# Tezahc/image_processor_pipeline

Measured on AMD Instinct MI355X. Metric: Mpixels/sec through 5-stage pipe, 1024×1024 uint8; achieved HBM GB/s, higher is better.
Workload: dtype u8

## Files before the change

### image_processor_pipeline_amd/_native.py

```python
from __future__ import annotations

import ctypes
import os
from pathlib import Path

import numpy as np

LIB_PATH = Path(os.environ.get("IPP_LIB_PATH", str(Path(__file__).resolve().parent / "libipp.so")))
_EXPERIMENT = os.environ.get("IPP_AB_EXPERIMENT") == "1"

IPP_OK = 0
IPP_E_ARG = -1
IPP_E_LAUNCH = -2
IPP_E_RANGE = -3
IPP_MAX_HSV_RANGES = 16
IPP_TAPS_MFMA = 1
IPP_RS_PREMULTIPLY = 1
IPP_RS_UNPREMULTIPLY = 2


class NativeUnavailable(RuntimeError):
    """The HIP C-ABI library could not be loaded (never silently bypassed)."""


class NativeError(RuntimeError):
    pass


_I4 = np.int32
_I8 = np.int64

GATHER_DESC = np.dtype([
    ("src_off", _I8), ("dst_off", _I8), ("src_pitch", _I4), ("src_cn", _I4),
    ("src_w", _I4), ("src_h", _I4), ("in_x0", _I4), ("in_y0", _I4), ("in_w", _I4), ("in_h", _I4),
    ("a0", _I4), ("a1", _I4), ("a2", _I4), ("a3", _I4), ("a4", _I4), ("a5", _I4),
    ("out_w", _I4), ("out_h", _I4), ("off_x", _I4), ("off_y", _I4), ("flip", _I4), ("dst_pitch", _I4),
    ("base_off", _I8), ("lim", np.uint32), ("b", _I4, (6,)), ("prepared", _I4),
], align=True)

AFFINE_DESC = np.dtype([
    ("src_off", _I8), ("dst_off", _I8), ("src_pitch", _I4), ("src_cn", _I4),
    ("in_x0", _I4), ("in_y0", _I4), ("in_w", _I4), ("in_h", _I4),
    ("out_w", _I4), ("out_h", _I4), ("dst_pitch", _I4), ("flip", _I4), ("m", np.float64, (6,)),
], align=True)

IPP_ENH_BLUR = 1
IPP_ENH_LUT = 2
ENHANCE_DESC = np.dtype([
    ("src_off", _I8), ("dst_off", _I8), ("w", _I4), ("h", _I4), ("src_pitch", _I4), ("dst_pitch", _I4),
    ("f_brightness", np.float32), ("f_contrast", np.float32), ("f_color", np.float32), ("flags", _I4),
    ("box_r", _I4), ("box_ww", np.uint32), ("box_fw", np.uint32), ("pad_", _I4), ("lut_off", _I8),
], align=True)

COPY_DESC = np.dtype([
    ("src_off", _I8), ("dst_off", _I8), ("src_pitch", _I4), ("dst_pitch", _I4),
    ("x0", _I4), ("y0", _I4), ("w", _I4), ("h", _I4), ("cn", _I4), ("flip", _I4),
], align=True)

HSV_RANGE = np.dtype([("lo", _I4, (3,)), ("hi", _I4, (3,)), ("zone", _I4, (4,))], align=True)
HSV_PARAMS = np.dtype([("n_ranges", _I4), ("bgr", _I4), ("r", HSV_RANGE, (IPP_MAX_HSV_RANGES,))], align=True)

IMAGE_DESC = np.dtype([("off", _I8), ("w", _I4), ("h", _I4), ("pitch", _I4), ("cn", _I4)], align=True)

CCL_WORK = np.dtype([("mask_off", _I8), ("edge_off", _I8), ("p_off", _I8), ("a_off", _I8), ("ent_off", _I8), ("ent_cap", _I8),
                     ("tile_off", _I8), ("img_off", _I8)], align=True)

RESAMPLE_DESC = np.dtype([
    ("src_off", _I8), ("dst_off", _I8), ("src_pitch", _I4), ("dst_pitch", _I4),
    ("in_len", _I4), ("out_len", _I4), ("lines", _I4), ("line0", _I4), ("ksize", _I4), ("pad_", _I4),
    ("coef_off", _I8),
], align=True)

PASTE_DESC = np.dtype([
    ("bg_off", _I8), ("ov_off", _I8), ("dst_off", _I8),
    ("bg_w", _I4), ("bg_h", _I4), ("bg_pitch", _I4), ("dst_pitch", _I4),
    ("ov_w", _I4), ("ov_h", _I4), ("ov_pitch", _I4), ("x", _I4), ("y", _I4), ("pad_", _I4),
], align=True)

PIPE_DESC = np.dtype([("g", GATHER_DESC), ("h", RESAMPLE_DESC), ("v", RESAMPLE_DESC), ("p", PASTE_DESC)],
                     align=True)

PIPE_PLAN_CFG = np.dtype([
    ("src_h", _I4), ("src_w", _I4), ("src_pitch", _I4), ("crop_t", _I4), ("crop_b", _I4), ("crop_l", _I4),
    ("crop_r", _I4), ("bg_h", _I4), ("bg_w", _I4), ("n_bg", _I4), ("n_sym", _I4), ("sym_flip", _I4, (4,)),
    ("n_global", _I4), ("start", _I4), ("stop", _I4), ("given", _I4), ("n_threads", _I4),
    ("ring_cols", _I4), ("pad_", _I4), ("seed", np.uint64),
    ("angle_min", np.float64), ("angle_max", np.float64), ("scale_min", np.float64), ("scale_max", np.float64),
], align=True)

PIPE_ITEM = np.dtype([
    ("angle", np.float64), ("ratio", np.float64), ("sym", _I4), ("bg_index", _I4), ("x", _I4), ("y", _I4),
    ("rot_w", _I4), ("rot_h", _I4), ("cut_x", _I4), ("cut_y", _I4), ("cut_w", _I4), ("cut_h", _I4),
    ("ov_w", _I4), ("ov_h", _I4),
], align=True)

TAP_AXIS = np.dtype([
    ("in_size", _I4), ("out_size", _I4), ("identity", _I4), ("shift", _I4), ("phase", _I4), ("nkb", _I4),
    ("compact", _I4), ("n_tiles", _I4), ("coef_off", _I8),
], align=True)

IPP_PLAN_TOTALS = 16
IPP_PIPE_COPY_GROUP = 8
IPP_PIPE_MAX_OV_W = 992
IPP_SCENE_MAP_MAX_LAYERS = 8
IPP_CONTOUR_HDR = 8
IPP_SIMPLIFY_LDS_VERTS = 2048
IPP_SIMPLIFY_THREADS = 256
PT = dict(coef_words=0, tmp_bytes=1, max_out_w=2, max_rows=3, max_ov_w=4, max_ov_h=5, algo_h=6, algo_v=7,
          copy_bytes=8, max_tiles=9, err_item=10, err_code=11, copy_reads=12)

_P = ctypes.c_void_p
_I = ctypes.c_int32
_L = ctypes.c_int64
_D = ctypes.c_double
SIGNATURES = {
    "ipp_rotate_flip_nearest": (_I, [_P, _P, _P, _I, _I, _I, _P]),
    "ipp_gather_prepare": (_I, [_P, _I]),
    "ipp_rotate_bilinear": (_I, [_P, _P, _P, _I, _I, _I, _P]),
    "ipp_copy_window": (_I, [_P, _P, _P, _I, _I, _I, _P]),
    "ipp_crop_to_bbox": (_I, [_P, _P, _P, _P, _I, _I, _I, _I, _P]),
    "ipp_hsv_mask": (_I, [_P, _P, _P, _P, _I, _I, _I, _P, _P]),
    "ipp_lanczos_h": (_I, [_P, _P, _P, _P, _I, _I, _I, _I, _P]),
    "ipp_lanczos_v": (_I, [_P, _P, _P, _P, _I, _I, _I, _I, _P]),
    "ipp_paste_blend": (_I, [_P, _P, _P, _P, _I, _I, _I, _P]),
    "ipp_pipe_hpass_bgcopy": (_I, [_P, _P, _P, _P, _I, _I, _I, _I, _P, _I, _P, _P, _P]),
    "ipp_pipe_vblend_bands": (_I, [_P, _P, _P, _P, _P, _I, _I, _I, _I, _I, _I, _P]),
    "ipp_ccl_keep_largest": (_I, [_P, _P, _I, _I, _I, _P, _P, _L, _P, _P, _P, _P]),
    "ipp_ccl_scratch_layout": (_L, [_I, _I, _P]),
    "ipp_video_keep_largest": (_I, [_P, _P, _I, _I, _I, _P, _P, _P, _L, _P, _P, _P, _P, _P, _P]),
    "ipp_alpha_bbox": (_I, [_P, _P, _I, _I, _I, _P, _P]),
    "ipp_alpha_bbox_min": (_I, [_P, _P, _I, _I, _I, _I, _P, _P]),
    "ipp_pipe_overlay_bbox": (_I, [_P, _P, _P, _I, _I, _I, _I, _I, _P, _P]),
    "ipp_pipe_hpass": (_I, [_P, _P, _P, _P, _I, _I, _I, _I, _P, _I, _P]),
    "ipp_pipe_vblend_over": (_I, [_P, _P, _P, _P, _I, _I, _I, _I, _I, _I, _P]),
    "ipp_pipe_scene_scratch_bytes": (_L, [_I, _I, _I, _I, _I]),
    "ipp_pipe_scene_boxes": (_I, [_P, _P, _P, _P, _I, _I, _I, _I, _I, _I, _I, _I, _P, _P, _P]),
    "ipp_pipe_scene_map": (_I, [_P, _P, _P, _P, _I, _I, _I, _I, _I, _I, _I, _I, _I, _I, _P, _P, _P, _L, _P]),
    "ipp_scene_contours_scratch_bytes": (_L, [_I, _I]),
    "ipp_scene_contours": (_I, [_P, _L, _I, _I, _P, _P, _I, _I, _I, _I, _P, _P, _P]),
    "ipp_scene_contours_pack": (_I, [_P, _P, _P, _I, _I, _P, _P]),
    "ipp_polygons_simplify_scratch_bytes": (_L, [_I, _L]),
    "ipp_polygons_simplify": (_I, [_P, _P, _P, _I, _L, _I, _I, _I, _P, _P, _P]),
    "ipp_polygons_simplify_pack": (_I, [_P, _P, _P, _P, _P, _P, _I, _P, _P]),
    "ipp_plan_lanczos": (_L, [_I, _D, _D, _I, _P, _L]),
    "ipp_plan_lanczos_ksize": (_I, [_D, _D, _I]),
    "ipp_plan_lanczos_batch": (_I, [_I, _P, _P, _P, _P, _L, _I]),
    "ipp_plan_opaque_bbox": (_I, [_I, _I, _P, _I, _I, _P]),
    "ipp_plan_mfma_size": (_L, [_I, _I, _I]),
    "ipp_plan_mfma_from_taps": (_I, [_I, _I, _I, _P, _I, _I, _P]),
    "ipp_plan_mfma_nk_bound": (_I, [_I, _I, _I]),
    "ipp_plan_pipe_axes": (_I, [_I, _P, _P, _P, _P, _P, _P, _P, _P, _I]),
    "ipp_stream_copy": (_I, [_P, _P, _L, _P]),
    "ipp_enhance_lsum": (_I, [_P, _P, _I, _L, _P, _P]),
    "ipp_enhance_color": (_I, [_P, _P, _P, _I, _L, _P, _P, _P]),
    "ipp_box_pass": (_I, [_P, _P, _P, _I, _L, _P, _I, _P, _I, _P]),
    "ipp_pipe_status": (_I, [_P, _P]),
    "ipp_plan_pipe_batch": (_I, [_P, _P, _P, _P, _P]),
    "ipp_pipe_taps_scratch_bytes": (_L, [_I]),
    "ipp_pipe_plan_taps": (_I, [_P, _I, _P, _P, _P, _P]),
    "ipp_pipe_plan_taps_cap": (_I, [_P, _I, _P, _P, _P, _L, _P]),
    "ipp_plan_mfma_tile": (_I, [_P, _I, _P, _P, _P, _L]),
    "ipp_plan_opaque_bbox_fast": (_I, [_I, _I, _P, _I, _I, _P]),
    "ipp_plan_py_hypot": (_D, [_D, _D]),
    "ipp_plan_rotation": (_I, [_I, _I, _D, _P]),
    "ipp_plan_py_random": (_I, [ctypes.c_uint64, _I, _P]),
    "ipp_version": (ctypes.c_char_p, []),
}

_lib = None


def load() -> ctypes.CDLL:
    global _lib
    if _lib is not None:
        return _lib
    if not LIB_PATH.exists():
        raise NativeUnavailable(
            f"{LIB_PATH} not found — build it with `make` or __graft_entry__.build(); "
            "there is no CPU fallback for the hot path")
    try:
        lib = ctypes.CDLL(str(LIB_PATH), mode=os.RTLD_NOW | getattr(os, "RTLD_LOCAL", 0))
    except OSError as e:
        raise NativeUnavailable(f"cannot load {LIB_PATH}: {e}") from e
    skipped = []
    for name, (res, args) in SIGNATURES.items():
        if _EXPERIMENT and not hasattr(lib, name):
            skipped.append(name)
            continue
        fn = getattr(lib, name)
        fn.restype = res
        fn.argtypes = args
    if skipped:
        import sys
        print(f"_native: IPP_AB_EXPERIMENT: {LIB_PATH} lacks {', '.join(skipped)}", file=sys.stderr)
    _lib = lib
    return lib


def check(rc: int, what: str) -> None:
    if rc != IPP_OK:
        raise NativeError(f"{what} failed with code {rc}")


def np_ptr(a: np.ndarray) -> int:
    return a.ctypes.data
```

### image_processor_pipeline_amd/csrc/ipp_label.hip

```cpp
#include <climits>

#include "ipp_device.h"
#include "ipp_pipe_layout.h"

namespace {

using namespace pipe_layout;

__global__ void k_label_bbox_init(int32_t* bbox, int n) {
    const int i = blockIdx.x * blockDim.x + threadIdx.x;
    if (i < n) {
        bbox[4 * i + 0] = INT32_MAX;
        bbox[4 * i + 1] = INT32_MAX;
        bbox[4 * i + 2] = -1;
        bbox[4 * i + 3] = -1;
    }
}

__global__ void k_label_bbox_finish(int32_t* bbox, int n) {
    const int i = blockIdx.x * blockDim.x + threadIdx.x;
    if (i < n && bbox[4 * i + 2] < 0) bbox[4 * i + 0] = bbox[4 * i + 1] = -1;
}

__device__ __forceinline__ void bbox_commit(int32_t* __restrict__ row, int xmin, int ymin, int xmax, int ymax) {
    for (int off = 32; off > 0; off >>= 1) {
        xmin = min(xmin, __shfl_xor(xmin, off));
        ymin = min(ymin, __shfl_xor(ymin, off));
        xmax = max(xmax, __shfl_xor(xmax, off));
        ymax = max(ymax, __shfl_xor(ymax, off));
    }
    if ((threadIdx.x & 63) == 0 && xmax >= 0) {
        atomicMin(&row[0], xmin);
        atomicMin(&row[1], ymin);
        atomicMax(&row[2], xmax + 1);
        atomicMax(&row[3], ymax + 1);
    }
}

template <typename Sink>
__device__ __forceinline__ void overlay_alpha_band(const uint8_t* __restrict__ tmp, const int32_t* __restrict__ coefs,
                                                   const ipp_pipe_desc* __restrict__ descs, int im, int ty,
                                                   Sink sink) {
    const ipp_paste_desc p = descs[im].p;
    int vb0, vb1;
    paste_bands(p, vb0, vb1);
    const int y0 = vb0 + ty * kBandRows;
    if (y0 >= vb1 || y0 >= p.bg_h) return;
    const int nrows = min(kBandRows, p.bg_h - y0);
    const int oy_lo = max(0, y0 - p.y), oy_hi = min(p.ov_h, y0 + nrows - p.y);
    if (oy_lo >= oy_hi) return;
    const int lane = threadIdx.x & 63;
    const int wave = __builtin_amdgcn_readfirstlane(threadIdx.x >> 6);

    const ipp_resample_desc v = descs[im].v;
    const int phase = tap_phase(p.y);
    const int t = band_tap_tile(y0, p.y, phase);
    const TapTiles tt = tap_tiles(coefs, v.coef_off, tap_ntiles(v.out_len, phase));
    int4 th = tt.hdr[t];
    th.x = __builtin_amdgcn_readfirstlane(th.x);
    th.y = __builtin_amdgcn_readfirstlane(th.y);
    th.z = __builtin_amdgcn_readfirstlane(th.z);
    const int ctiles = (p.ov_w + 15) >> 4;
    const int64_t gstride = t_pitch_vecs(v.src_pitch);
    const int x_l = lane & 15;
    int32_t rb[4];
#pragma unroll
    for (int r = 0; r < 4; ++r) rb[r] = tt.bias[kBiasWords * t + 4 * (lane >> 4) + r];
    const int gbase = t_row_group(th.x + 16 * (lane >> 4));
    const uint8_t* abase = tmp + v.src_off + gbase * gstride * kTGroupBytes + kTAlphaByte;

    for (int ct = wave; ct < ctiles; ct += 4) {
        const int x = 16 * ct + x_l;
        const int xs = min(x, p.ov_w - 1);
        const uint8_t* aq = abase + (int64_t)xs * kTGroupBytes;
        i32x4 acc[3];
        acc[0] = i32x4{rb[0], rb[1], rb[2], rb[3]};
        acc[1] = i32x4{0, 0, 0, 0};
        acc[2] = i32x4{0, 0, 0, 0};
#pragma unroll 1
        for (int ks = 0; ks < th.y; ++ks) {
            i32x4 bq;
#pragma unroll
            for (int j = 0; j < 4; ++j)
                bq[j] = *reinterpret_cast<const int32_t*>(aq + (kKStepGroups * ks + j) * gstride * kTGroupBytes);
#pragma unroll
            for (int q = 0; q < 3; ++q) {
                const i32x4 a = __builtin_bit_cast(i32x4, tt.blk[th.z + tap_dense_block(ks, q, lane)]);
                acc[q] = __builtin_amdgcn_mfma_i32_16x16x64_i8(a, bq, acc[q], 0, 0, 0);
            }
        }
#pragma unroll
        for (int r = 0; r < 4; ++r) {
            const int32_t s = planes3(acc[0][r], acc[1][r], acc[2][r]);
            const int32_t a = min(max(s >> 22, 0), 255);
            const int o = y0 + 4 * (lane >> 4) + r - p.y;
            if (x < p.ov_w && o >= oy_lo && o < oy_hi) sink(x, o, a);
        }
    }
}

__global__ void __launch_bounds__(256)
k_pipe_overlay_bbox(const uint8_t* __restrict__ tmp, const int32_t* __restrict__ coefs,
                    const ipp_pipe_desc* __restrict__ descs, FastDiv tiles_y, int alpha_min,
                    int32_t* __restrict__ bbox) {
    const uint32_t b = xcd_remap(blockIdx.x, gridDim.x);
    const int im = (int)fdiv(b, tiles_y);
    const int ty = (int)(b - (uint32_t)im * tiles_y.d);
    int xmin = INT32_MAX, ymin = INT32_MAX, xmax = -1, ymax = -1;
    overlay_alpha_band(tmp, coefs, descs, im, ty, [&](int x, int o, int a) {
        if (a >= alpha_min) {
            xmin = min(xmin, x);
            xmax = max(xmax, x);
            ymin = min(ymin, o);
            ymax = max(ymax, o);
        }
    });
    bbox_commit(bbox + 4 * (int64_t)im, xmin, ymin, xmax, ymax);
}

constexpr int BT_W = 64, BT_H = 16, BT_PX = 4;

__global__ void __launch_bounds__(256)
k_alpha_bbox_min(const uint8_t* __restrict__ img, const ipp_image_desc* __restrict__ descs, int tiles_x,
                 int tiles_y, int alpha_min, int32_t* __restrict__ bbox) {
    const uint32_t b = xcd_remap(blockIdx.x, gridDim.x);
    const int per_img = tiles_x * tiles_y;
    const int im = b / per_img;
    const int t = b - im * per_img;
    const int ty = t / tiles_x, tx = t - ty * tiles_x;
    const ipp_image_desc d = descs[im];
    const int y = ty * BT_H + (int)(threadIdx.x >> 4);
    const int x0 = tx * BT_W + (int)(threadIdx.x & 15) * BT_PX;
    int xmin = INT32_MAX, ymin = INT32_MAX, xmax = -1, ymax = -1;
    if (y < d.h && (d.cn == 2 || d.cn == 4)) {
        const uint8_t* row = img + d.off + (int64_t)y * d.pitch;
        for (int k = 0; k < BT_PX; ++k) {
            const int x = x0 + k;
            if (x < d.w && (int)row[(int64_t)x * d.cn + d.cn - 1] >= alpha_min) {
                xmin = min(xmin, x);
                xmax = max(xmax, x);
                ymin = min(ymin, y);
                ymax = max(ymax, y);
            }
        }
    }
    bbox_commit(bbox + 4 * (int64_t)im, xmin, ymin, xmax, ymax);
}

__host__ __device__ constexpr int64_t scene_pitch(int max_ov_w) { return ((int64_t)max_ov_w + 15) & ~(int64_t)15; }
__host__ __device__ constexpr int64_t scene_table_bytes(int64_t slots) { return (4 * slots + 255) & ~(int64_t)255; }

__global__ void k_scene_init(int32_t* __restrict__ out, int32_t* __restrict__ table,
                             const int32_t* __restrict__ scene_layer, int n, int n_scenes, int K) {
    const int i = blockIdx.x * blockDim.x + threadIdx.x;
    if (i >= n) return;
    out[6 * i + 0] = INT32_MAX;
    out[6 * i + 1] = INT32_MAX;
    out[6 * i + 2] = -1;
    out[6 * i + 3] = -1;
    out[6 * i + 4] = 0;
    out[6 * i + 5] = 0;
    const int s = scene_layer[2 * i], k = scene_layer[2 * i + 1];
    if ((unsigned)s < (unsigned)n_scenes && (unsigned)k < (unsigned)K) table[(int64_t)s * K + k] = i;
}

__global__ void k_scene_finish(int32_t* out, int n) {
    const int i = blockIdx.x * blockDim.x + threadIdx.x;
    if (i < n && out[6 * i + 2] < 0) out[6 * i + 0] = out[6 * i + 1] = -1;
}

__global__ void __launch_bounds__(256)
k_scene_alpha(const uint8_t* __restrict__ tmp, const int32_t* __restrict__ coefs,
              const ipp_pipe_desc* __restrict__ descs, FastDiv tiles_y, int max_ov_w, int max_ov_h,
              uint8_t* __restrict__ planes) {
    const uint32_t b = xcd_remap(blockIdx.x, gridDim.x);
    const int im = (int)fdiv(b, tiles_y);
    const int ty = (int)(b - (uint32_t)im * tiles_y.d);
    if (descs[im].p.ov_w > max_ov_w || descs[im].p.ov_h > max_ov_h) return;
    const int64_t pitch = scene_pitch(max_ov_w);
    uint8_t* plane = planes + (int64_t)im * max_ov_h * pitch;
    overlay_alpha_band(tmp, coefs, descs, im, ty,
                       [&](int x, int o, int a) { plane[(int64_t)o * pitch + x] = (uint8_t)a; });
}

constexpr int SVR = 16;

__global__ void __launch_bounds__(256)
k_scene_visible(const ipp_pipe_desc* __restrict__ descs, const int32_t* __restrict__ scene_layer,
                const int32_t* __restrict__ table, const uint8_t* __restrict__ planes, FastDiv strips, int n,
                int n_scenes, int K, int max_ov_w, int max_ov_h, int alpha_min, int cover_min,
                int32_t* __restrict__ out) {
    const uint32_t b = xcd_remap(blockIdx.x, gridDim.x);
    const int im = (int)fdiv(b, strips);
    const int v0 = (int)(b - (uint32_t)im * strips.d) * SVR;
    const ipp_paste_desc p = descs[im].p;
    if (v0 >= p.ov_h || p.ov_w > max_ov_w || p.ov_h > max_ov_h) return;
    const int64_t pitch = scene_pitch(max_ov_w), psize = (int64_t)max_ov_h * pitch;
    const uint8_t* plane = planes + (int64_t)im * psize;
    const int scene = scene_layer[2 * im], layer = scene_layer[2 * im + 1];
    const bool mapped = (unsigned)scene < (unsigned)n_scenes && (unsigned)layer < (unsigned)K;
    const int v = v0 + (int)(threadIdx.x >> 4);
    int xmin = INT32_MAX, ymin = INT32_MAX, xmax = -1, ymax = -1, area = 0, vis = 0;
    for (int u0 = 4 * (int)(threadIdx.x & 15); u0 < p.ov_w; u0 += 64) {
        uint32_t a4 = 0u;
        if (v < p.ov_h) a4 = *reinterpret_cast<const uint32_t*>(plane + (int64_t)v * pitch + u0);
        uint32_t present = 0u;
#pragma unroll
        for (int k = 0; k < 4; ++k)
            present |= (uint32_t)(v < p.ov_h && u0 + k < p.ov_w && (int)((a4 >> (8 * k)) & 255u) >= alpha_min) << k;
        uint32_t hidden = 0u;
        for (int j = mapped ? layer + 1 : K; j < K; ++j) {
            const int dj = table[(int64_t)scene * K + j];
            if ((unsigned)dj >= (unsigned)n) continue;
            const ipp_paste_desc q = descs[dj].p;
            if (q.ov_w > max_ov_w || q.ov_h > max_ov_h) continue;
            const int cy = p.y + v - q.y;
            if ((unsigned)cy >= (unsigned)q.ov_h) continue;
            const uint8_t* qrow = planes + (int64_t)dj * psize + (int64_t)cy * pitch;
#pragma unroll
            for (int k = 0; k < 4; ++k) {
                const int cx = p.x + u0 + k - q.x;
                if (((present >> k) & 1u) && (unsigned)cx < (unsigned)q.ov_w && (int)qrow[cx] >= cover_min)
                    hidden |= 1u << k;
            }
        }
        const uint32_t visible = present & ~hidden;
        area += __builtin_popcount(present);
        vis += __builtin_popcount(visible);
        if (visible) {
            xmin = min(xmin, p.x + u0 + (int)__builtin_ctz(visible));
            xmax = max(xmax, p.x + u0 + 31 - (int)__builtin_clz(visible));
            ymin = min(ymin, p.y + v);
            ymax = max(ymax, p.y + v);
        }
    }
    for (int off = 32; off > 0; off >>= 1) {
        area += __shfl_xor(area, off);
        vis += __shfl_xor(vis, off);
    }
    int32_t* row = out + 6 * (int64_t)im;
    bbox_commit(row, xmin, ymin, xmax, ymax);
    if ((threadIdx.x & 63) == 0) {
        if (area) atomicAdd(&row[4], area);
        if (vis) atomicAdd(&row[5], vis);
    }
}

constexpr int MT_W = 256, MT_H = 16, MT_PX = 16;
constexpr int kSceneMapMaxLayers = IPP_SCENE_MAP_MAX_LAYERS;
static_assert(kSceneMapMaxLayers == 8, "one bit per layer in a map byte");
static_assert(MT_PX == 16 && MT_W == 16 * MT_PX && MT_H * (MT_W / MT_PX) == 256, "k_scene_map's thread map");

__global__ void k_scene_table(int32_t* __restrict__ table, const int32_t* __restrict__ scene_layer, int n,
                              int n_scenes, int K) {
    const int i = blockIdx.x * blockDim.x + threadIdx.x;
    if (i >= n) return;
    const int s = scene_layer[2 * i], k = scene_layer[2 * i + 1];
    if ((unsigned)s < (unsigned)n_scenes && (unsigned)k < (unsigned)K) table[(int64_t)s * K + k] = i;
}

__global__ void __launch_bounds__(256)
k_scene_map(const ipp_pipe_desc* __restrict__ descs, const int32_t* __restrict__ table,
            const uint8_t* __restrict__ planes, FastDiv tiles, FastDiv tiles_x, int n, int K, int bg_w, int bg_h,
            int max_ov_w, int max_ov_h, int alpha_min, int cover_min, uint8_t* __restrict__ map,
            int64_t map_pitch) {
    const uint32_t b = xcd_remap(blockIdx.x, gridDim.x);
    const int scene = (int)fdiv(b, tiles);
    const uint32_t t = b - (uint32_t)scene * tiles.d;
    const int ty = (int)fdiv(t, tiles_x), tx = (int)(t - (uint32_t)ty * tiles_x.d);
    const int bx0 = tx * MT_W;
    const int wy0 = ty * MT_H + 4 * __builtin_amdgcn_readfirstlane((int)(threadIdx.x >> 6));
    const int Y = ty * MT_H + (int)(threadIdx.x >> 4);
    const int X0 = bx0 + MT_PX * (int)(threadIdx.x & 15);
    const int64_t pitch = scene_pitch(max_ov_w), psize = (int64_t)max_ov_h * pitch;

    int d[kSceneMapMaxLayers], px[kSceneMapMaxLayers], py[kSceneMapMaxLayers], pw[kSceneMapMaxLayers],
        ph[kSceneMapMaxLayers];
#pragma unroll
    for (int k = 0; k < kSceneMapMaxLayers; ++k) {
        d[k] = -1;
        px[k] = py[k] = pw[k] = ph[k] = 0;
        if (k >= K) continue;
        const int dk = table[(int64_t)scene * K + k];
        if ((unsigned)dk >= (unsigned)n) continue;
        const ipp_paste_desc p = descs[dk].p;
        if (p.ov_w <= 0 || p.ov_h <= 0 || p.ov_w > max_ov_w || p.ov_h > max_ov_h) continue;
        const int64_t rx0 = max((int64_t)p.x, (int64_t)0), rx1 = min((int64_t)p.x + p.ov_w, (int64_t)bg_w);
        const int64_t ry0 = max((int64_t)p.y, (int64_t)0), ry1 = min((int64_t)p.y + p.ov_h, (int64_t)bg_h);
        if (rx0 >= (int64_t)bx0 + MT_W || rx1 <= bx0 || ry0 >= (int64_t)wy0 + 4 || ry1 <= wy0) continue;
        d[k] = dk;
        px[k] = p.x, py[k] = p.y, pw[k] = p.ov_w, ph[k] = p.ov_h;
    }

    if (Y >= bg_h || X0 >= map_pitch) return;
    uint32_t w[4] = {0u, 0u, 0u, 0u};
    uint32_t covered = 0u;
#pragma unroll
    for (int k = kSceneMapMaxLayers - 1; k >= 0; --k) {
        if (d[k] < 0) continue;
        const int cy = Y - py[k];
        if ((unsigned)cy >= (unsigned)ph[k]) continue;
        const uint8_t* row = planes + (int64_t)d[k] * psize + (int64_t)cy * pitch;
        const int cx0 = X0 - px[k];
        const int xlim = min(pw[k], bg_w - px[k]);
#pragma unroll
        for (int i = 0; i < MT_PX; ++i) {
            const int cx = cx0 + i;
            if (cx >= 0 && cx < xlim) {
                const int a = row[cx];
                if (!((covered >> i) & 1u) && a >= alpha_min) w[i >> 2] |= (1u << k) << (8 * (i & 3));
                if (a >= cover_min) covered |= 1u << i;
            }
        }
    }
    store16<0>(map + ((int64_t)scene * bg_h + Y) * map_pitch + X0, 16, true, w);
}

int scene_launches(const uint8_t* tmp, const int32_t* coefs, const ipp_pipe_desc* descs, const int32_t* scene_layer,
                   int n_images, int n_scenes, int per_scene, int bg_w, int bg_h, int max_ov_w, int max_ov_h,
                   int alpha_min, int cover_min, uint8_t* scratch, int32_t* rows, uint8_t* map, int64_t map_pitch,
                   hipStream_t s) {
    const int tyb = paste_max_bands(max_ov_h), strips = (max_ov_h + SVR - 1) / SVR;
    const int64_t slots = (int64_t)n_scenes * per_scene;
    if ((int64_t)tyb * n_images >= INT32_MAX || (int64_t)strips * n_images >= INT32_MAX || slots >= INT32_MAX)
        return IPP_E_ARG;
    int mtx = 0, mty = 0;
    if (map) {
        mtx = (int)((map_pitch + MT_W - 1) / MT_W), mty = (bg_h + MT_H - 1) / MT_H;
        if ((int64_t)mtx * mty * n_scenes >= INT32_MAX) return IPP_E_ARG;
    }
    int32_t* table = reinterpret_cast<int32_t*>(scratch);
    uint8_t* planes = scratch + scene_table_bytes(slots);
    if (slots > 0 && hipMemsetAsync(table, 0xFF, 4 * (size_t)slots, s) != hipSuccess) return IPP_E_LAUNCH;
    if (n_images > 0) {
        const int ib = (n_images + 255) / 256;
        if (rows)
            hipLaunchKernelGGL(k_scene_init, dim3(ib), dim3(256), 0, s, rows, table, scene_layer, n_images, n_scenes,
                               per_scene);
        else
            hipLaunchKernelGGL(k_scene_table, dim3(ib), dim3(256), 0, s, table, scene_layer, n_images, n_scenes,
                               per_scene);
        hipLaunchKernelGGL(k_scene_alpha, dim3((uint32_t)(tyb * n_images)), dim3(256), 0, s, tmp, coefs, descs,
                           fast_div((uint32_t)tyb), max_ov_w, max_ov_h, planes);
        if (rows) {
            hipLaunchKernelGGL(k_scene_visible, dim3((uint32_t)(strips * n_images)), dim3(256), 0, s, descs,
                               scene_layer, table, planes, fast_div((uint32_t)strips), n_images, n_scenes, per_scene,
                               max_ov_w, max_ov_h, alpha_min, cover_min, rows);
            hipLaunchKernelGGL(k_scene_finish, dim3(ib), dim3(256), 0, s, rows, n_images);
        }
    }
    if (map && n_scenes > 0)
        hipLaunchKernelGGL(k_scene_map, dim3((uint32_t)(mtx * mty * n_scenes)), dim3(256), 0, s, descs, table, planes,
                           fast_div((uint32_t)(mtx * mty)), fast_div((uint32_t)mtx), n_images, per_scene, bg_w, bg_h,
                           max_ov_w, max_ov_h, alpha_min, cover_min, map, map_pitch);
    IPP_CHECK_LAUNCH();
    return IPP_OK;
}

}

extern "C" int ipp_pipe_overlay_bbox(const uint8_t* tmp, const int32_t* coefs, const ipp_pipe_desc* descs,
                                     int32_t n_images, int32_t max_ov_w, int32_t max_ov_h, int32_t alpha_min,
                                     int32_t tap_format, int32_t* bbox, void* stream) {
    if (alpha_min < 1 || alpha_min > 255 || tap_format != IPP_TAPS_MFMA) return IPP_E_ARG;
    if (!tmp || !coefs || !descs || !bbox || n_images < 0 || max_ov_w <= 0 || max_ov_h <= 0) return IPP_E_ARG;
    if (n_images == 0) return IPP_OK;
    const int tyb = paste_max_bands(max_ov_h);
    const int64_t nb = (int64_t)tyb * n_images;
    if (nb >= INT32_MAX) return IPP_E_ARG;
    hipStream_t s = (hipStream_t)stream;
    const int ib = (n_images + 255) / 256;
    hipLaunchKernelGGL(k_label_bbox_init, dim3(ib), dim3(256), 0, s, bbox, n_images);
    hipLaunchKernelGGL(k_pipe_overlay_bbox, dim3((uint32_t)nb), dim3(256), 0, s, tmp, coefs, descs,
                       fast_div((uint32_t)tyb), alpha_min, bbox);
    hipLaunchKernelGGL(k_label_bbox_finish, dim3(ib), dim3(256), 0, s, bbox, n_images);
    IPP_CHECK_LAUNCH();
    return IPP_OK;
}

extern "C" int ipp_alpha_bbox_min(const uint8_t* img, const ipp_image_desc* descs, int32_t n_images,
                                  int32_t max_w, int32_t max_h, int32_t alpha_min, int32_t* bbox, void* stream) {
    if (alpha_min < 1 || alpha_min > 255) return IPP_E_ARG;
    if (!img || !descs || !bbox || n_images < 0 || max_w <= 0 || max_h <= 0) return IPP_E_ARG;
    if (n_images == 0) return IPP_OK;
    const int tx = (max_w + BT_W - 1) / BT_W, ty = (max_h + BT_H - 1) / BT_H;
    const int64_t blocks = (int64_t)tx * ty * n_images;
    if (blocks >= (int64_t)INT32_MAX) return IPP_E_ARG;
    hipStream_t s = (hipStream_t)stream;
    const int ib = (n_images + 255) / 256;
    hipLaunchKernelGGL(k_label_bbox_init, dim3(ib), dim3(256), 0, s, bbox, n_images);
    hipLaunchKernelGGL(k_alpha_bbox_min, dim3((uint32_t)blocks), dim3(256), 0, s, img, descs, tx, ty, alpha_min,
                       bbox);
    hipLaunchKernelGGL(k_label_bbox_finish, dim3(ib), dim3(256), 0, s, bbox, n_images);
    IPP_CHECK_LAUNCH();
    return IPP_OK;
}

extern "C" int64_t ipp_pipe_scene_scratch_bytes(int32_t n_images, int32_t n_scenes, int32_t per_scene,
                                                int32_t max_ov_w, int32_t max_ov_h) {
    if (n_images < 0 || n_scenes < 0 || per_scene < 1 || max_ov_w <= 0 || max_ov_h <= 0) return IPP_E_ARG;
    return scene_table_bytes((int64_t)n_scenes * per_scene) + (int64_t)n_images * max_ov_h * scene_pitch(max_ov_w);
}

extern "C" int ipp_pipe_scene_boxes(const uint8_t* tmp, const int32_t* coefs, const ipp_pipe_desc* descs,
                                    const int32_t* scene_layer, int32_t n_images, int32_t n_scenes,
                                    int32_t per_scene, int32_t max_ov_w, int32_t max_ov_h, int32_t alpha_min,
                                    int32_t cover_min, int32_t tap_format, uint8_t* scratch, int32_t* out,
                                    void* stream) {
    if (alpha_min < 1 || alpha_min > 255 || cover_min < 1 || cover_min > 255 || tap_format != IPP_TAPS_MFMA)
        return IPP_E_ARG;
    if (!tmp || !coefs || !descs || !scene_layer || !scratch || !out || n_images < 0 || n_scenes < 0 ||
        per_scene < 1 || max_ov_w <= 0 || max_ov_h <= 0)
        return IPP_E_ARG;
    if ((reinterpret_cast<uintptr_t>(scratch) & 15u) != 0) return IPP_E_ARG;
    if (n_images == 0) return IPP_OK;
    return scene_launches(tmp, coefs, descs, scene_layer, n_images, n_scenes, per_scene, 0, 0, max_ov_w, max_ov_h,
                          alpha_min, cover_min, scratch, out, nullptr, 0, (hipStream_t)stream);
}

extern "C" int ipp_pipe_scene_map(const uint8_t* tmp, const int32_t* coefs, const ipp_pipe_desc* descs,
                                  const int32_t* scene_layer, int32_t n_images, int32_t n_scenes, int32_t per_scene,
                                  int32_t bg_w, int32_t bg_h, int32_t max_ov_w, int32_t max_ov_h, int32_t alpha_min,
                                  int32_t cover_min, int32_t tap_format, uint8_t* scratch, int32_t* rows,
                                  uint8_t* map, int64_t map_pitch, void* stream) {
    if (alpha_min < 1 || alpha_min > 255 || cover_min < 1 || cover_min > 255 || tap_format != IPP_TAPS_MFMA)
        return IPP_E_ARG;
    if (!tmp || !coefs || !descs || !scene_layer || !scratch || !map || n_images < 0 || n_scenes < 0 ||
        per_scene < 1 || per_scene > IPP_SCENE_MAP_MAX_LAYERS || max_ov_w <= 0 || max_ov_h <= 0)
        return IPP_E_ARG;
    if (bg_w <= 0 || bg_h <= 0 || map_pitch < bg_w || (map_pitch & 15) != 0 || map_pitch > INT32_MAX)
        return IPP_E_ARG;
    if (((reinterpret_cast<uintptr_t>(scratch) | reinterpret_cast<uintptr_t>(map)) & 15u) != 0) return IPP_E_ARG;
    return scene_launches(tmp, coefs, descs, scene_layer, n_images, n_scenes, per_scene, bg_w, bg_h, max_ov_w,
                          max_ov_h, alpha_min, cover_min, scratch, rows, map, map_pitch, (hipStream_t)stream);
}
```

### image_processor_pipeline_amd/csrc/ipp_pipe.hip

```cpp
#include <algorithm>
#include <type_traits>

#include "ipp_hsv.h"
#include "ipp_pipe_layout.h"
#include "ipp_sampler.h"

namespace {

using namespace pipe_layout;

constexpr int HR = 16;
constexpr int RING = 512;
constexpr int WSTRIDE = 544;

__device__ __forceinline__ uint32_t perm(uint32_t hi, uint32_t lo, uint32_t sel) {
    return __builtin_amdgcn_perm(hi, lo, sel);
}

__device__ __forceinline__ void transpose4(uint32_t p0, uint32_t p1, uint32_t p2, uint32_t p3, uint32_t ch[4]) {
    const uint32_t lo01 = perm(p1, p0, 0x05010400u), hi01 = perm(p1, p0, 0x07030602u);
    const uint32_t lo23 = perm(p3, p2, 0x05010400u), hi23 = perm(p3, p2, 0x07030602u);
    ch[0] = perm(lo23, lo01, 0x05040100u);
    ch[1] = perm(lo23, lo01, 0x07060302u);
    ch[2] = perm(hi23, hi01, 0x05040100u);
    ch[3] = perm(hi23, hi01, 0x07060302u);
}

__device__ __forceinline__ __amdgpu_buffer_rsrc_t rsrc_of(const void* p) {
    return __builtin_amdgcn_make_buffer_rsrc(const_cast<void*>(p), (short)0, 0x7FFFFFFF, 0x00020000);
}

typedef uint8_t WinRing[4][HR][WSTRIDE];

template <int NR>
struct __attribute__((aligned(16))) Hpass2Lds {
    WinRing win;
    HsvTables<NR> T;
    int32_t zc[NR > 8 ? 2 * NR : 1];
};

template <int NR, bool ZONES>
__device__ __forceinline__ uint32_t hsv2_px(const HsvTables<NR>& T, uint32_t raw, uint32_t zbits) {
    uint32_t ex = hsv_tab_excl<NR, false>(T, raw);
    if (ZONES) ex &= zbits;
    const uint32_t t = (raw | 0xFF000000u) ^ 0x80808080u;
    return ex ? 0x80808080u : t;
}

struct Hp2Block {
    u32x4_t rsv;
    uint32_t lim;
    uint32_t rowx, rowy;
    int32_t b0, b3, pitch, in_w, in_h;
    int32_t xlo, xhi;
};

struct Raw4 {
    uint32_t p[4];
    uint32_t fl;
    bool any;
    bool live;
};

__device__ __forceinline__ uint32_t asm_gather(u32x4_t rs, uint32_t off) {
    uint32_t v;
    asm volatile("buffer_load_dword %0, %1, %2, 0 offen" : "=v"(v) : "v"(off), "s"(rs));
    return v;
}
__device__ __forceinline__ void asm_wait(uint32_t (&p)[4], int32_t newer) {
    asm volatile(
        "; gather wait %0 %1 %2 %3\n\t"
        "s_cmp_eq_u32 %4, 8\n\t"
        "s_cbranch_scc0 1f\n\t"
        "s_waitcnt vmcnt(8)\n\t"
        "s_branch 4f\n"
        "1:\n\t"
        "s_cmp_eq_u32 %4, 4\n\t"
        "s_cbranch_scc0 2f\n\t"
        "s_waitcnt vmcnt(4)\n\t"
        "s_branch 4f\n"
        "2:\n\t"
        "s_cmp_eq_u32 %4, 0\n\t"
        "s_cbranch_scc0 4f\n\t"
        "s_waitcnt vmcnt(0)\n"
        "4:"
        : "+v"(p[0]), "+v"(p[1]), "+v"(p[2]), "+v"(p[3])
        : "s"(newer)
        : "scc");
}

template <int CN, bool CLAMP>
__device__ __forceinline__ void hp2_issue(const Hp2Block& B, uint32_t xx, uint32_t yy, Raw4& o) {
    bool any = false;
    uint32_t off[4];
    if (CLAMP) o.fl = 0u;
#pragma unroll
    for (int k = 0; k < 4; ++k) {
        const int xin = (int32_t)xx >> 16, yin = (int32_t)yy >> 16;
        const bool ok = CLAMP ? ((uint32_t)xin < (uint32_t)B.in_w) & ((uint32_t)yin < (uint32_t)B.in_h)
                              : (uint32_t)xin < (uint32_t)B.in_w;
        uint32_t o1 = (uint32_t)__mul24(yin, B.pitch) + (uint32_t)__umul24((uint32_t)xin, (uint32_t)CN);
        if (CLAMP) {
            const uint32_t offc = min(o1, B.lim);
            o.fl |= (uint32_t)(o1 != offc) << (1 + k);
            o1 = offc;
        }
        off[k] = ok ? o1 : 0xFFFFFFFFu;
        any |= ok;
        xx += (uint32_t)B.b0;
        yy += (uint32_t)B.b3;
    }
#pragma unroll
    for (int k = 0; k < 4; ++k) o.p[k] = asm_gather(B.rsv, off[k]);
    o.any = any;
    o.live = true;
}

constexpr int HP_NW = 4;
constexpr int HP_STEPC = 16 * HP_NW;

__device__ int32_t g_pipe_status;

struct Hp2Chunk {
    int s0, s1;
    int c0;
    int ng4;
    int nsteps;
};

__device__ __forceinline__ Hp2Chunk hp2_chunk(const int4* hdr, int s0, int ntiles, int& filled, int wave) {
    Hp2Chunk c;
    c.s0 = s0;
    int4 hh[4];
#pragma unroll
    for (int k = 0; k < 4; ++k) hh[k] = hdr[s0 + k];
    const int W0 = hh[0].x;
    int W1 = hh[0].x + 64 * hh[0].y, s1 = s0 + 1;
    if (W1 - W0 > RING && threadIdx.x == 0) atomicOr(&g_pipe_status, 1);
    bool grow = true;
#pragma unroll
    for (int k = 1; k < 4; ++k) {
        const int e = max(W1, hh[k].x + 64 * hh[k].y);
        grow = grow && s0 + k < ntiles && e - W0 <= RING;
        if (grow) {
            W1 = e;
            s1 = s0 + k + 1;
        }
    }
    c.s1 = s1;
    c.c0 = max(filled, W0);
    c.ng4 = max(0, (W1 - c.c0) >> 2);
    c.nsteps = c.ng4 > wave * 4 ? (c.ng4 - wave * 4 + 4 * HP_NW - 1) / (4 * HP_NW) : 0;
    filled = max(filled, W1);
    return c;
}

template <int NR, bool ZONES, int CN, bool CLAMP>
__device__ __forceinline__ void hpass2_body(const HsvTables<NR>& T, WinRing& win, int wave, const Hp2Block& B,
                                            uint8_t* __restrict__ tmp, const int32_t* __restrict__ coefs,
                                            const ipp_resample_desc& h, int row0, int nrows, const int32_t* zc0,
                                            const int32_t* zcw, uint32_t zrow, int s_lo, int s_hi) {
    const int lane = threadIdx.x & 63;
    const int r = 2 * (lane >> 3) + ((lane >> 1) & 1);
    const int ntiles = (h.out_len + kTileOut - 1) >> kTileOutLog2;
    const int4* hdr = reinterpret_cast<const int4*>(coefs + h.coef_off);
    const int32_t* tbias = coefs + h.coef_off + kHdrWords * (int64_t)ntiles;
    const uint4* tblk = reinterpret_cast<const uint4*>(coefs + h.coef_off + (kHdrWords + kBiasWords) * (int64_t)ntiles);
    const uint32_t sx = (uint32_t)HP_STEPC * (uint32_t)B.b0, sy = (uint32_t)HP_STEPC * (uint32_t)B.b3;

    int filled = hdr[s_lo].x;
    Hp2Chunk ck = hp2_chunk(hdr, s_lo, s_hi, filled, wave);
    auto lane_x = [&](const Hp2Chunk& c) { return c.c0 + 16 * wave + 8 * ((lane >> 2) & 1) + 4 * (lane & 1); };
    int xl = lane_x(ck);
    uint32_t xxl = B.rowx + (uint32_t)__mul24(xl, B.b0), yyl = B.rowy + (uint32_t)__mul24(xl, B.b3);
    Raw4 RA, RB, RC;
    RA.live = RB.live = RC.live = false;
    RA.fl = RB.fl = RC.fl = 0u;
    auto issue = [&](const Hp2Chunk& c, int st, uint32_t xx, uint32_t yy, Raw4& o) {
        const int xs = c.c0 + 16 * wave + HP_STEPC * st;
        const bool live = st < c.nsteps && xs + 15 >= B.xlo && xs <= B.xhi;
        if (!live) {
            o.any = false;
            o.live = false;
            return;
        }
        hp2_issue<CN, CLAMP>(B, xx, yy, o);
    };
    issue(ck, 0, xxl, yyl, RA);
    issue(ck, 1, xxl + sx, yyl + sy, RB);
    __syncthreads();
    const uint32_t fill = __builtin_amdgcn_readfirstlane(hsv2_px<NR, ZONES>(T, 0u, ~0u));

    for (;;) {
        const int t = ck.s0 + wave;
        const bool has_tile = t < ck.s1 && nrows > 0;
        int4 th = make_int4(0, 0, 0, 0);
        uint4 bn[3];
        int32_t meta = 0;
        int32_t bias = 0;
        {
            const int te = min(t, s_hi - 1);
            th = hdr[te];
            th.x = __builtin_amdgcn_readfirstlane(th.x);
            th.y = __builtin_amdgcn_readfirstlane(th.y);
            th.z = __builtin_amdgcn_readfirstlane(th.z);
            th.w = __builtin_amdgcn_readfirstlane(th.w);
#pragma unroll
            for (int p = 0; p < kTapPlanes; ++p)
                bn[p] = tblk[th.z + (th.w ? kCompactMeta : 0) + lane + p * kKStepCols];
            if (!has_tile) th.y = 0;
        }
        const int te = min(t, s_hi - 1);

        const int c0 = ck.c0, ng4 = ck.ng4, nsteps = ck.nsteps;
        auto process = [&](Raw4& P, int st, int newer) {
            asm_wait(P.p, P.live ? newer : -1);
            const int cg = wave * 4 + 4 * HP_NW * st + 2 * ((lane >> 2) & 1) + (lane & 1);
            const int x = c0 + 4 * cg;
            const bool active = (cg < ng4) && (r < nrows);
            uint32_t px[4], zb[4];
#pragma unroll
            for (int k = 0; k < 4; ++k) {
                zb[k] = ~0u;
                if (ZONES) {
                    const int xk = x + k;
                    zb[k] = 0;
#pragma unroll
                    for (int q = 0; q < NR; ++q) zb[k] |= (uint32_t)((uint32_t)(xk - zc0[q]) < (uint32_t)zcw[q]) << q;
                    zb[k] &= zrow;
                }
            }
            uint32_t ch[4];
            if (__builtin_amdgcn_ballot_w64(P.any) != 0ull) {
#pragma unroll
                for (int k = 0; k < 4; ++k) {
                    uint32_t raw = P.p[k];
                    if (CLAMP) raw >>= ((P.fl >> (1 + k)) & 1u) << 3;
                    px[k] = hsv2_px<NR, ZONES>(T, raw, zb[k]);
                }
                transpose4(px[0], px[1], px[2], px[3], ch);
            } else if (ZONES) {
#pragma unroll
                for (int k = 0; k < 4; ++k) px[k] = hsv2_px<NR, ZONES>(T, 0u, zb[k]);
                transpose4(px[0], px[1], px[2], px[3], ch);
            } else {
#pragma unroll
                for (int c = 0; c < 4; ++c) ch[c] = ((fill >> (8 * c)) & 0xFFu) * 0x01010101u;
            }
            if (active) {
                const int pos = x & (RING - 1);
#pragma unroll
                for (int c = 0; c < 4; ++c) *reinterpret_cast<uint32_t*>(&win[c][r][pos]) = ch[c];
            }
        };
        auto iss = [&](int st2, Raw4& o) { issue(ck, st2, xxl + st2 * sx, yyl + st2 * sy, o); };
        bool mb = false;
        for (int st = 0; st < nsteps; st += 3) {
            iss(st + 2, RC);
            if (st + 3 >= nsteps) {
                meta = reinterpret_cast<const int32_t*>(tblk + th.z)[lane & 15];
                bias = tbias[min(kBiasWords * te + (lane & 15), h.out_len - 1)];
                mb = true;
            }
            process(RA, st, 4 * (RB.live + RC.live));
            iss(st + 3, RA);
            process(RB, st + 1, 4 * (RC.live + RA.live));
            iss(st + 4, RB);
            process(RC, st + 2, 4 * (RA.live + RB.live));
        }

        if (!mb) {
            meta = reinterpret_cast<const int32_t*>(tblk + th.z)[lane & 15];
            bias = tbias[min(kBiasWords * te + (lane & 15), h.out_len - 1)];
        }
        const int s1 = ck.s1;
        const bool more = s1 < s_hi;
        if (more) {
            ck = hp2_chunk(hdr, s1, s_hi, filled, wave);
            xl = lane_x(ck);
            xxl = B.rowx + (uint32_t)__mul24(xl, B.b0);
            yyl = B.rowy + (uint32_t)__mul24(xl, B.b3);
        } else {
            ck.nsteps = 0;
        }
        asm volatile("" ::"v"(bn[0].x), "v"(bn[1].x), "v"(bn[2].x), "v"(bias), "v"(meta));
        issue(ck, 0, xxl, yyl, RA);
        issue(ck, 1, xxl + sx, yyl + sy, RB);
        __syncthreads();

        if (has_tile) {
            i32x4 acc[4][3];
            const int32_t b0 = bias - (128 << 22);
#pragma unroll
            for (int c = 0; c < 4; ++c) {
                acc[c][0] = i32x4{b0, b0, b0, b0};
                acc[c][1] = i32x4{0, 0, 0, 0};
                acc[c][2] = i32x4{0, 0, 0, 0};
            }
            const int arow = lane & 15, akoff = 16 * (lane >> 4);
            if (th.w) {
#pragma unroll 1
                for (int ks = 0; ks < th.y; ++ks) {
                    const int rel = 4 * ks + (lane >> 4) - (meta & 0xFF);
                    const bool ok = (unsigned)rel < (unsigned)((meta >> 8) & 0xFF);
                    const int src = ((meta >> 16) + rel) << 2;
                    const int pos = (th.x + 64 * ks + akoff) & (RING - 1);
#pragma unroll
                    for (int p = 0; p < 3; ++p) {
                        const uint32_t w[4] = {bn[p].x, bn[p].y, bn[p].z, bn[p].w};
                        i32x4 bq;
#pragma unroll
                        for (int d = 0; d < 4; ++d) {
                            const int v = __builtin_amdgcn_ds_bpermute(src, (int)w[d]);
                            bq[d] = ok ? v : 0;
                        }
#pragma unroll
                        for (int c = 0; c < 4; ++c) {
                            const i32x4 av = *reinterpret_cast<const i32x4*>(&win[c][arow][pos]);
                            acc[c][p] = __builtin_amdgcn_mfma_i32_16x16x64_i8(av, bq, acc[c][p], 0, 0, 0);
                        }
                    }
                }
            } else {
#pragma unroll 1
                for (int ks = 0; ks < th.y; ++ks) {
                    if (ks > 0) {
#pragma unroll
                        for (int p = 0; p < kTapPlanes; ++p) bn[p] = tblk[th.z + lane + (ks * kTapPlanes + p) * kKStepCols];
                    }
                    const int pos = (th.x + 64 * ks + akoff) & (RING - 1);
#pragma unroll
                    for (int c = 0; c < 4; ++c) {
                        const i32x4 av = *reinterpret_cast<const i32x4*>(&win[c][arow][pos]);
#pragma unroll
                        for (int p = 0; p < 3; ++p)
                            acc[c][p] = __builtin_amdgcn_mfma_i32_16x16x64_i8(av, __builtin_bit_cast(i32x4, bn[p]),
                                                                            acc[c][p], 0, 0, 0);
                    }
                }
            }
            const int xo = 16 * t + (lane & 15);
            if (xo < h.out_len) {
                uint32_t outc[4];
#pragma unroll
                for (int c = 0; c < 4; ++c) {
                    int32_t ss[4];
#pragma unroll
                    for (int rr = 0; rr < 4; ++rr) ss[rr] = planes3(acc[c][0][rr], acc[c][1][rr], acc[c][2][rr]);
                    outc[c] = clip8x4_x80(ss[0], ss[1], ss[2], ss[3]);
                }
                int ln = lane;
                asm volatile("" : "+v"(ln));
                const int grp = (row0 >> kTGroupRowsLog2) + (ln >> 4);
                TGroup* dst = reinterpret_cast<TGroup*>(tmp + h.dst_off + (int64_t)grp * h.dst_pitch) + xo;
                const uint32_t w[4] = {outc[0], outc[1], outc[2], outc[3]};
                store16<2>(reinterpret_cast<uint8_t*>(dst), kTGroupBytes, true, w);
            }
        }
        asm_wait(RA.p, RA.live ? 4 * RB.live : -1);
        asm_wait(RB.p, RB.live ? 0 : -1);
        if (!more) break;
        __syncthreads();
    }
}

__device__ __forceinline__ bool band_cols_split(const ipp_paste_desc& p, const uint8_t* bg, const uint8_t* dst,
                                                int& gx0, int& gx1) {
    return pipe_layout::band_cols_split(p, gx0, gx1, [&] {
        return ((reinterpret_cast<uintptr_t>(bg + p.bg_off) | reinterpret_cast<uintptr_t>(dst + p.dst_off)) & 15u) == 0;
    });
}

constexpr int kCopyU = 16;
template <int NT = 256, int U = kCopyU>
__device__ __forceinline__ void bg_copy_outside_bands(const ipp_paste_desc& p, const uint8_t* __restrict__ bg,
                                                      uint8_t* __restrict__ dst, int share, int nshare) {
    int vb0, vb1;
    paste_bands(p, vb0, vb1);
    const int rb = 3 * p.bg_w;
    const uint8_t* sb = bg + p.bg_off;
    uint8_t* db = dst + p.dst_off;
    const bool flat = p.bg_pitch == rb && p.dst_pitch == rb && (rb & 15) == 0 &&
                      ((reinterpret_cast<uintptr_t>(sb) | reinterpret_cast<uintptr_t>(db)) & 15u) == 0;
    if (flat) {
        int gx0, gx1;
        const bool split = band_cols_split(p, bg, dst, gx0, gx1);
        const int L = split ? 3 * gx0 : 0, LR = split ? 3 * ((p.bg_w >> 4) - gx1) + L : 0;
        const int rv = rb / 16, rgt = 3 * gx1 - L;
        const uint32_t mag = LR > 0 ? (uint32_t)((0x100000000ull + LR - 1) / LR) : 0u;
        const int64_t n0 = (int64_t)vb0 * rb / 16, n1 = (int64_t)(p.bg_h - vb1) * rb / 16;
        const int64_t n2 = (int64_t)(vb1 - vb0) * LR, V = n0 + n1 + n2;
        const int64_t a = V * share / nshare, e = V * (share + 1) / nshare;
        const int64_t skip = (int64_t)vb1 * rb / 16 - n0;
        auto vec_of = [&](int64_t i) -> int64_t {
            if (i < n0) return i;
            if (i < n0 + n1) return i + skip;
            const uint32_t j = (uint32_t)(i - n0 - n1);
            const uint32_t r = __umulhi(j, mag), c = j - r * (uint32_t)LR;
            return (int64_t)(vb0 + (int)r) * rv + (int)c + ((int)c < L ? 0 : rgt);
        };
        const u32x4_t* s4 = reinterpret_cast<const u32x4_t*>(sb);
        u32x4_t* d4 = reinterpret_cast<u32x4_t*>(db);
        for (int64_t i0 = a + threadIdx.x; i0 < e; i0 += U * NT) {
            u32x4_t v[U];
#pragma unroll
            for (int j = 0; j < U; ++j) {
                const int64_t i = i0 + NT * j;
                if (i < e) v[j] = s4[vec_of(i)];
            }
#pragma unroll
            for (int j = 0; j < U; ++j) {
                const int64_t i = i0 + NT * j;
                if (i < e) __builtin_nontemporal_store(v[j], d4 + vec_of(i));
            }
        }
        return;
    }
    const int R = vb0 + (p.bg_h - vb1);
    const int ra = (int)((int64_t)R * share / nshare), re = (int)((int64_t)R * (share + 1) / nshare);
    const int chunks = (rb + 15) >> 4;
    for (int rr = ra; rr < re; ++rr) {
        const int y = rr < vb0 ? rr : rr - vb0 + vb1;
        const uint8_t* brow = sb + (int64_t)y * p.bg_pitch;
        uint8_t* drow = db + (int64_t)y * p.dst_pitch;
        for (int ci = threadIdx.x; ci < chunks; ci += NT) {
            const int c0 = ci << 4, nb = min(16, rb - c0);
            const bool vec = nb == 16 && ((reinterpret_cast<uintptr_t>(brow + c0) | reinterpret_cast<uintptr_t>(drow + c0)) & 15u) == 0;
            uint32_t w[4];
            load16(brow + c0, nb, vec, w);
            store16<2>(drow + c0, nb, vec, w);
        }
    }
}

#ifndef IPP_COPY_GROUP
#define IPP_COPY_GROUP IPP_PIPE_COPY_GROUP
#endif
#ifndef IPP_COPY_SLABS
#define IPP_COPY_SLABS IPP_COPY_GROUP
#endif
constexpr int kCopyGU = 4;
constexpr int kCopyGroup = IPP_COPY_GROUP;
constexpr int kCopySlabs = IPP_COPY_SLABS;
static_assert(kCopyGroup >= 1 && kCopyGroup <= 64, "one lane per item of a copy group");

struct CopyItem {
    uint32_t dlo, dhi;
    uint32_t blo, bhi;
    int32_t dims;
    int32_t vb0, vb1;
    int32_t c0, c1;
    int32_t flat;
};

template <int NT = 256, int U = kCopyGU>
__device__ __forceinline__ void bg_copy_group(const ipp_pipe_desc* __restrict__ descs, int n, int i0, int slab,
                                              const uint8_t* __restrict__ bg, uint8_t* __restrict__ dst) {
    const int cnt = min(kCopyGroup, n - i0);
    if (cnt <= 0) return;
    const int lane = threadIdx.x & 63;
    CopyItem ci = {0u, 0u, 0u, 0u, -1, 0, 0, 0, 0, 0};
    if (lane < cnt) {
        const ipp_paste_desc& p = descs[i0 + lane].p;
        const int rb = 3 * p.bg_w;
        const uint8_t* sb = bg + p.bg_off;
        uint8_t* db = dst + p.dst_off;
        const uint64_t du = reinterpret_cast<uint64_t>(db), bu = reinterpret_cast<uint64_t>(sb);
        ci.dlo = (uint32_t)du;
        ci.dhi = (uint32_t)(du >> 32);
        ci.blo = (uint32_t)bu;
        ci.bhi = (uint32_t)(bu >> 32);
        ci.dims = p.bg_w | (p.bg_h << 16);
        int vb0, vb1, gx0, gx1;
        paste_bands(p, vb0, vb1);
        ci.vb0 = vb0;
        ci.vb1 = vb1;
        const bool split = band_cols_split(p, bg, dst, gx0, gx1);
        ci.c0 = split ? 3 * gx0 : 0;
        ci.c1 = split ? 3 * gx1 : rb / 16;
        const int64_t rv = rb / 16, slab_rows = (p.bg_h + kCopySlabs - 1) / kCopySlabs;
        ci.flat = p.bg_pitch == rb && p.dst_pitch == rb && (rb & 15) == 0 && ((du | bu) & 15u) == 0 &&
                  p.bg_w < 65536 && p.bg_h < 32768 && slab_rows * rv * rv < (1ll << 32);
    }
    auto rl = [](int32_t v, int j) { return __builtin_amdgcn_readlane(v, j); };
    auto rlu = [](uint32_t v, int j) { return (uint32_t)__builtin_amdgcn_readlane((int32_t)v, j); };
    int j0 = 0;
    while (j0 < cnt) {
        const uint32_t blo = rlu(ci.blo, j0), bhi = rlu(ci.bhi, j0);
        const int32_t dims = rl(ci.dims, j0);
        int j1 = j0 + 1;
        while (j1 < cnt && rlu(ci.blo, j1) == blo && rlu(ci.bhi, j1) == bhi && rl(ci.dims, j1) == dims) ++j1;
        uint64_t fm = 0;
        for (int j = j0; j < j1; ++j) fm |= (uint64_t)(rl(ci.flat, j) != 0) << j;
        if (fm) {
            const int bw = dims & 0xFFFF, bh = dims >> 16;
            const int rv = 3 * bw / 16;
            const int ya = (int)((int64_t)bh * slab / kCopySlabs), ye = (int)((int64_t)bh * (slab + 1) / kCopySlabs);
            const uint32_t total = (uint32_t)((ye - ya) * rv);
            const uint32_t mag = (uint32_t)((0x100000000ull + rv - 1) / rv);
            const u32x4_t* s4 = reinterpret_cast<const u32x4_t*>(((uint64_t)bhi << 32) | blo) + (int64_t)ya * rv;
            for (uint32_t ib = threadIdx.x; ib < total; ib += U * NT) {
                u32x4_t v[U];
                uint32_t rc[U];
#pragma unroll
                for (int u = 0; u < U; ++u) {
                    const uint32_t i = ib + NT * u;
                    const uint32_t q = __umulhi(i, mag);
                    rc[u] = (q << 16) | (i - q * (uint32_t)rv);
                    if (i < total) v[u] = s4[i];
                }
                for (int j = j0; j < j1; ++j) {
                    if (!((fm >> j) & 1u)) continue;
                    const int32_t r0 = rl(ci.vb0, j) - ya, rn = rl(ci.vb1, j) - rl(ci.vb0, j);
                    const int32_t c0 = rl(ci.c0, j), cn = rl(ci.c1, j) - c0;
                    u32x4_t* d4 = reinterpret_cast<u32x4_t*>(((uint64_t)rlu(ci.dhi, j) << 32) | rlu(ci.dlo, j)) +
                                  (int64_t)ya * rv;
#pragma unroll
                    for (int u = 0; u < U; ++u) {
                        const uint32_t i = ib + NT * u;
                        const bool inside = (uint32_t)((int32_t)(rc[u] >> 16) - r0) < (uint32_t)rn &&
                                            (uint32_t)((int32_t)(rc[u] & 0xFFFFu) - c0) < (uint32_t)cn;
                        if (i < total && !inside) __builtin_amdgcn_raw_buffer_store_b128(v[u], rsrc_of(d4), i * 16u, 0, 2);
                    }
                }
            }
        }
        for (int j = j0; j < j1; ++j)
            if (!((fm >> j) & 1u)) bg_copy_outside_bands<NT>(descs[i0 + j].p, bg, dst, slab, kCopySlabs);
        j0 = j1;
    }
}

__device__ __forceinline__ bool yr_range_ok(int in_h, int pitch, int need) {
    return (int64_t)in_h * pitch >= (int64_t)need && (int64_t)32768 * pitch + need <= (int64_t)1 << 32;
}

template <int NR, bool ZONES, int CN>
__device__ __forceinline__ void hpass_block(Hpass2Lds<NR>& L, const uint8_t* __restrict__ src,
                                            uint8_t* __restrict__ tmp, const int32_t* __restrict__ coefs,
                                            const ipp_pipe_desc* __restrict__ descs, int im, int tb,
                                            const ipp_hsv_params& hp) {
    const ipp_gather_desc g = descs[im].g;
    const ipp_resample_desc h = descs[im].h;
    const int row0 = tb * HR;
    if (row0 >= h.lines) return;
    const int wave = __builtin_amdgcn_readfirstlane(threadIdx.x >> 6);

    hsv_tables_init<NR>(L.T, hp);

    int32_t zc0r[ZONES && NR <= 8 ? NR : 1], zcwr[ZONES && NR <= 8 ? NR : 1];
    int32_t* zc0 = zc0r;
    int32_t* zcw = zcwr;
    if (ZONES && NR > 8) {
        zc0 = L.zc;
        zcw = L.zc + NR;
    }
    uint32_t zrow = 0;
    const int lane = threadIdx.x & 63;
    const int y = h.line0 + row0 + 2 * (lane >> 3) + ((lane >> 1) & 1);
    if (ZONES) {
#pragma unroll
        for (int k = 0; k < NR; ++k) {
            int a, bb, cc, dd;
            slice_indices(hp.r[k].zone[0], g.out_h - hp.r[k].zone[1], g.out_h, a, bb);
            slice_indices(hp.r[k].zone[2], g.out_w - hp.r[k].zone[3], g.out_w, cc, dd);
            zrow |= (uint32_t)(y >= a && y < bb) << k;
            if (NR <= 8 || threadIdx.x == 0) {
                zc0[k] = cc;
                zcw[k] = dd - cc;
            }
        }
    }

    const Sampler S = make_sampler(src, g);
    const int nrec = (g.src_h - g.in_y0) * g.src_pitch - g.in_x0 * g.src_cn;
    const int need = (g.in_h - 1) * g.src_pitch + g.in_w * CN + (CN == 3 ? 1 : 0);
    const bool fast = need <= nrec && yr_range_ok(g.in_h, (int)S.pitch, need);
    const uint64_t sbu = reinterpret_cast<uint64_t>(S.base);
    Hp2Block B;
    B.rsv = u32x4_t{(uint32_t)sbu, (uint32_t)(sbu >> 32) & 0xFFFFu, (uint32_t)(fast ? min(nrec, need) : nrec),
                    0x00020000u};
    B.lim = S.lim;
    B.rowx = (uint32_t)S.b2 + (uint32_t)y * (uint32_t)S.b1;
    B.rowy = (uint32_t)S.b5 + (uint32_t)y * (uint32_t)S.b4;
    B.b0 = S.b0;
    B.b3 = S.b3;
    B.pitch = (int32_t)S.pitch;
    B.in_w = S.in_w;
    B.in_h = S.in_h;
    {
        float lo = -1e9f, hi = 1e9f;
        auto clip = [&](float a, float bb, float lim) {
            if (bb == 0.0f) {
                if (!(a >= 0.0f && a < lim)) { lo = 1e9f; hi = -1e9f; }
            } else {
                const float t1 = -a / bb, t2 = (lim - a) / bb;
                lo = fmaxf(lo, fminf(t1, t2));
                hi = fminf(hi, fmaxf(t1, t2));
            }
        };
        clip((float)(int32_t)B.rowx, (float)S.b0, 65536.0f * (float)S.in_w);
        clip((float)(int32_t)B.rowy, (float)S.b3, 65536.0f * (float)S.in_h);
        const int ilo = lo > hi ? 0x3FFFFFFF : (int)fmaxf(lo - 2.0f, -1e8f);
        const int ihi = lo > hi ? -0x3FFFFFFF : (int)fminf(hi + 2.0f, 1e8f);
        int blo = 0x3FFFFFFF, bhi = -0x3FFFFFFF;
#pragma unroll
        for (int rr = 0; rr < HR; ++rr) {
            const int lr = 8 * (rr >> 1) + 2 * (rr & 1);
            blo = min(blo, __builtin_amdgcn_readlane(ilo, lr));
            bhi = max(bhi, __builtin_amdgcn_readlane(ihi, lr));
        }
        B.xlo = blo;
        B.xhi = bhi;
    }

    const int ntiles = (h.out_len + kTileOut - 1) >> kTileOutLog2;
    int s_lo = 0, s_hi = ntiles;
    if constexpr (!ZONES) {
        bool black_out = false;
#pragma unroll
        for (int k = 0; k < NR; ++k) {
            const ipp_hsv_range& q = hp.r[k];
            black_out |= q.lo[0] <= 0 && q.hi[0] >= 0 && q.lo[1] <= 0 && q.hi[1] >= 0 && q.lo[2] <= 0 && q.hi[2] >= 0;
        }
        if (black_out && ntiles <= 64) {
            const int4* hdr = reinterpret_cast<const int4*>(coefs + h.coef_off);
            const int4 hv = hdr[min(lane, ntiles - 1)];
            const bool keep = lane < ntiles && hv.x + 64 * hv.y > B.xlo && hv.x <= B.xhi;
            const uint64_t km = __builtin_amdgcn_ballot_w64(keep);
            s_lo = km ? __builtin_ctzll(km) : 0;
            s_hi = km ? 64 - __builtin_clzll(km) : 0;
            const int ntrim = s_lo + ntiles - s_hi;
            for (int i = wave; i < ntrim; i += HP_NW) {
                const int t = i < s_lo ? i : i - s_lo + s_hi;
                const int xo = 16 * t + (lane & 15);
                if (xo < h.out_len) {
                    const int grp = (row0 >> kTGroupRowsLog2) + (lane >> 4);
                    TGroup* dst = reinterpret_cast<TGroup*>(tmp + h.dst_off + (int64_t)grp * h.dst_pitch) + xo;
                    const uint32_t w[4] = {0x80808080u, 0x80808080u, 0x80808080u, 0x80808080u};
                    store16<2>(reinterpret_cast<uint8_t*>(dst), kTGroupBytes, true, w);
                }
            }
            if (s_lo >= s_hi) return;
        }
    }

    const int nrows = min(HR, h.lines - row0);
    if (fast)
        hpass2_body<NR, ZONES, CN, false>(L.T, L.win, wave, B, tmp, coefs, h, row0, nrows, zc0, zcw, zrow, s_lo, s_hi);
    else
        hpass2_body<NR, ZONES, CN, true>(L.T, L.win, wave, B, tmp, coefs, h, row0, nrows, zc0, zcw, zrow, s_lo, s_hi);
}

template <int NR, bool ZONES, int CN>
__global__ void __launch_bounds__(64 * HP_NW) __attribute__((amdgpu_waves_per_eu(ZONES ? 3 : 4)))
k_pipe_hpass2(const uint8_t* __restrict__ src, uint8_t* __restrict__ tmp, const int32_t* __restrict__ coefs,
              const ipp_pipe_desc* __restrict__ descs, int n, FastDiv tiles_y, FastDiv per_grp, ipp_hsv_params hp,
              const uint8_t* __restrict__ bg, uint8_t* __restrict__ dst) {
    __shared__ Hpass2Lds<NR> L;
    const uint32_t b = xcd_remap(blockIdx.x, gridDim.x);
    const int ty = (int)tiles_y.d;
    const int grp = (int)fdiv(b, per_grp);
    const int t = (int)(b - (uint32_t)grp * per_grp.d);
    if (t >= kCopyGroup * ty) {
        bg_copy_group<64 * HP_NW>(descs, n, grp * kCopyGroup, t - kCopyGroup * ty, bg, dst);
        return;
    }
    const int j = (int)fdiv((uint32_t)t, tiles_y);
    const int im = grp * kCopyGroup + j;
    if (im >= n) return;
    hpass_block<NR, ZONES, CN>(L, src, tmp, coefs, descs, im, t - j * ty, hp);
}

#ifndef IPP_VB_DB
#define IPP_VB_DB 2
#endif
#ifndef IPP_VB_HOIST_MAX
#define IPP_VB_HOIST_MAX 3
#endif
#ifndef IPP_VB_WPE
#define IPP_VB_WPE 3
#endif

__host__ __device__ constexpr int orow_stride(int ov_w_max) { return (ov_w_max + 32 + 3) & ~3; }
static_assert((size_t)kBandRows * orow_stride(IPP_PIPE_MAX_OV_W) * 4 <= 64 * 1024, "V-pass rows in LDS");
static_assert((size_t)kBandRows * orow_stride(IPP_PIPE_MAX_OV_W + 1) * 4 > 64 * 1024, "IPP_PIPE_MAX_OV_W is the limit");

typedef unsigned short u16x2 __attribute__((ext_vector_type(2)));

__device__ __forceinline__ uint32_t blend_u16x2(uint32_t bg, uint32_t ov, uint32_t al) {
    const u16x2 b = __builtin_bit_cast(u16x2, bg), o = __builtin_bit_cast(u16x2, ov), a = __builtin_bit_cast(u16x2, al);
    const u16x2 c255 = {255, 255}, c128 = {128, 128}, c8 = {8, 8};
    const u16x2 t = (u16x2)(o - b) * a + (b * c255 + c128);
    return __builtin_bit_cast(uint32_t, (u16x2)((u16x2)(t + (t >> c8)) >> c8));
}

__device__ __forceinline__ void blend48(uint32_t (&bg)[12], const uint32_t (&ov)[16]) {
#pragma unroll
    for (int d = 0; d < 12; ++d) {
        uint32_t r[2];
#pragma unroll
        for (int h = 0; h < 2; ++h) {
            const int j0 = 4 * d + h, j1 = j0 + 2;
            const int p0 = j0 / 3, p1 = j1 / 3, c0 = j0 % 3, c1 = j1 % 3;
            const uint32_t sel_ov = (uint32_t)c0 | 0x0c00u | ((uint32_t)(p1 == p0 ? c1 : 4 + c1) << 16) | 0x0c000000u;
            const uint32_t sel_al = 3u | 0x0c00u | ((uint32_t)(p1 == p0 ? 3 : 7) << 16) | 0x0c000000u;
            const uint32_t ovp = __builtin_amdgcn_perm(ov[p1], ov[p0], sel_ov);
            const uint32_t alp = __builtin_amdgcn_perm(ov[p1], ov[p0], sel_al);
            const uint32_t bgp = __builtin_amdgcn_perm(0u, bg[d], h ? 0x0c030c01u : 0x0c020c00u);
            r[h] = blend_u16x2(bgp, ovp, alp);
        }
        bg[d] = __builtin_amdgcn_perm(r[1], r[0], 0x06020400u);
    }
}

__device__ __forceinline__ void horner8(i32x4& acc, int32_t a0, int32_t a1, int32_t a2, int32_t a3) {
    acc = (acc << 8) + i32x4{a0, a1, a2, a3};
}

__device__ __forceinline__ i32x4 vb_bop(const u32x4_t (&g)[4], int c) {
    return i32x4{(int)g[0][c], (int)g[1][c], (int)g[2][c], (int)g[3][c]};
}

template <int NK>
__device__ __forceinline__ void vb_mfma_tile(const i32x4 (&ta)[NK][3], const i32x4 (&bq)[NK][4], const int32_t (&rb)[4],
                                             i32x4 (&acc)[4]) {
#pragma unroll
    for (int c = 0; c < 4; ++c) acc[c] = i32x4{0, 0, 0, 0};
#pragma unroll
    for (int q = 2; q >= 0; --q) {
#pragma unroll
        for (int ks = 0; ks < NK; ++ks)
#pragma unroll
            for (int c = 0; c < 4; ++c) acc[c] = __builtin_amdgcn_mfma_i32_16x16x64_i8(ta[ks][q], bq[ks][c], acc[c], 0, 0, 0);
        if (q == 2) {
#pragma unroll
            for (int c = 0; c < 4; ++c) acc[c] <<= 8;
        } else if (q == 1) {
#pragma unroll
            for (int c = 0; c < 4; ++c) horner8(acc[c], rb[0], rb[1], rb[2], rb[3]);
        }
    }
}

template <bool INPLACE>
struct VbPtr {
    typedef const uint8_t* __restrict__ bg_t;
    typedef uint8_t* __restrict__ dst_t;
};
template <>
struct VbPtr<true> {
    typedef const uint8_t* bg_t;
    typedef uint8_t* dst_t;
};
__device__ __forceinline__ ipp_paste_desc vb_paste_desc(const ipp_paste_desc& q, bool inplace) {
    ipp_paste_desc p = q;
    if (inplace) {
        p.bg_off = p.dst_off;
        p.bg_pitch = p.dst_pitch;
    }
    return p;
}

template <bool MAGIC, bool INPLACE = false>
__device__ __forceinline__ void vblend_block(uint32_t* __restrict__ orow, const uint8_t* __restrict__ tmp,
                                             typename VbPtr<INPLACE>::bg_t bg, typename VbPtr<INPLACE>::dst_t dst,
                                             const int32_t* __restrict__ coefs,
                                             const ipp_pipe_desc* __restrict__ descs, int im, int ty, int ov_w_max) {
    const ipp_paste_desc p = vb_paste_desc(descs[im].p, INPLACE);
    int y0 = ty * kBandRows;
    {
        int vb0, vb1;
        paste_bands(p, vb0, vb1);
        y0 += vb0;
        if (y0 >= vb1) return;
    }
    if (y0 >= p.bg_h) return;
    const int nrows = min(kBandRows, p.bg_h - y0);
    const int oy_lo = max(0, y0 - p.y), oy_hi = min(p.ov_h, y0 + nrows - p.y);
    const bool any = oy_lo < oy_hi;
    const int lane = threadIdx.x & 63;
    const int wave = __builtin_amdgcn_readfirstlane(threadIdx.x >> 6);

    const int os = orow_stride(ov_w_max), xo = p.x & 15;
    const uint8_t* bgb = bg + p.bg_off + (int64_t)y0 * p.bg_pitch;
    uint8_t* dsb = dst + p.dst_off + (int64_t)y0 * p.dst_pitch;
    const bool groups = (p.bg_w & 15) == 0 && ((p.bg_pitch | p.dst_pitch) & 15) == 0 &&
                        ((reinterpret_cast<uintptr_t>(bgb) | reinterpret_cast<uintptr_t>(dsb)) & 15u) == 0;
    int sx0, sx1;
    const bool csplit = groups && band_cols_split(p, bg, dst, sx0, sx1);
    const int gc0 = csplit ? sx0 : 0;
    const int G = csplit ? sx1 - sx0 : p.bg_w >> 4, lg = 31 - __builtin_clz(max(G, 1));
    const bool pow2 = (G & (G - 1)) == 0;
    const int gtotal = nrows * G;
    auto gload = [&](int idx, uint4 (&v)[3]) {
        const int rr = pow2 ? idx >> lg : idx / G;
        const int gi = gc0 + idx - rr * G;
        const uint4* sp = reinterpret_cast<const uint4*>(bgb + (int64_t)rr * p.bg_pitch) + 3 * gi;
#pragma unroll
        for (int q = 0; q < 3; ++q) v[q] = sp[q];
    };
    uint4 gcur[3];
    if (any) {
        uint32_t* umag = orow + kBandRows * os;
        if (MAGIC) {
            umag[threadIdx.x] = unpremul_magic(threadIdx.x);
            __syncthreads();
        }
        for (int e = threadIdx.x; e < kBandRows * 32; e += 256) {
            const int row = e >> 5, c = e & 31;
            if (c < xo) orow[row * os + c] = 0u;
            else if (c >= 16) orow[row * os + xo + p.ov_w + c - 16] = 0u;
        }
        const ipp_resample_desc v = descs[im].v;
        const int phase = tap_phase(p.y);
        const int t = band_tap_tile(y0, p.y, phase);
        const TapTiles tt = tap_tiles(coefs, v.coef_off, tap_ntiles(v.out_len, phase));
        const int4 th = tt.hdr[t];
        const int ctiles = (p.ov_w + 15) >> 4;
        const int gstride = t_pitch_vecs(v.src_pitch);
        const int x_l = lane & 15;
        int32_t rb[4];
#pragma unroll
        for (int r = 0; r < 4; ++r) rb[r] = tt.bias[kBiasWords * t + 4 * (lane >> 4) + r];
        const u32x4_t* tbase = reinterpret_cast<const u32x4_t*>(tmp + v.src_off);
        const int gbase = t_row_group(th.x + 16 * (lane >> 4));
        auto tload = [&](int ct, int ks, u32x4_t (&g)[4]) {
            const int xs = min(16 * ct + x_l, p.ov_w - 1);
            const u32x4_t* tq = t_group(tbase, gstride, gbase + kKStepGroups * ks, xs);
#pragma unroll
            for (int j = 0; j < 4; ++j) g[j] = tq[j * gstride];
        };
        auto epilogue = [&](int ct, auto s) {
            const int x = 16 * ct + x_l;
            if (x < p.ov_w) {
#pragma unroll
                for (int r = 0; r < 4; ++r) {
                    const int row = 4 * (lane >> 4) + r;
                    const int o = y0 + row - p.y;
                    if (o >= oy_lo && o < oy_hi) {
                        const uint32_t px = clip8x4_mfma(s(0, r), s(1, r), s(2, r), s(3, r));
                        orow[row * os + xo + x] = MAGIC ? unpremultiply_magic(px, umag) : unpremultiply(px);
                    }
                }
            }
        };
        auto tiles = [&](auto nkc) {
            constexpr int NK = decltype(nkc)::value;
            if constexpr (NK > 0) {
                i32x4 ta[NK][3];
#pragma unroll
                for (int ks = 0; ks < NK; ++ks)
#pragma unroll
                    for (int q = 0; q < 3; ++q)
                        ta[ks][q] = __builtin_bit_cast(i32x4, tt.blk[th.z + tap_dense_block(ks, q, lane)]);
                auto transpose = [&](const u32x4_t (&g)[NK][4], i32x4 (&bq)[NK][4]) {
#pragma unroll
                    for (int ks = 0; ks < NK; ++ks)
#pragma unroll
                        for (int c = 0; c < 4; ++c) bq[ks][c] = vb_bop(g[ks], c);
                };
                if constexpr (NK <= IPP_VB_DB) {
                    i32x4 bc[NK][4];
                    u32x4_t gn[NK][4];
                    int ct = wave;
                    if (ct < ctiles) {
#pragma unroll
                        for (int ks = 0; ks < NK; ++ks) tload(ct, ks, gn[ks]);
                        transpose(gn, bc);
                    }
                    for (; ct < ctiles; ct += 4) {
                        const bool more = ct + 4 < ctiles;
                        if (more) {
#pragma unroll
                            for (int ks = 0; ks < NK; ++ks) tload(ct + 4, ks, gn[ks]);
                        }
                        i32x4 acc[4];
                        vb_mfma_tile<NK>(ta, bc, rb, acc);
                        epilogue(ct, [&](int c, int r) { return acc[c][r]; });
                        if (more) transpose(gn, bc);
                    }
                } else {
                    for (int ct = wave; ct < ctiles; ct += 4) {
                        u32x4_t g[NK][4];
#pragma unroll
                        for (int ks = 0; ks < NK; ++ks) tload(ct, ks, g[ks]);
                        i32x4 bq[NK][4];
                        transpose(g, bq);
                        i32x4 acc[4];
                        vb_mfma_tile<NK>(ta, bq, rb, acc);
                        epilogue(ct, [&](int c, int r) { return acc[c][r]; });
                    }
                }
            } else {
                for (int ct = wave; ct < ctiles; ct += 4) {
                    i32x4 acc[4][3];
#pragma unroll
                    for (int c = 0; c < 4; ++c) {
                        acc[c][0] = i32x4{rb[0], rb[1], rb[2], rb[3]};
                        acc[c][1] = i32x4{0, 0, 0, 0};
                        acc[c][2] = i32x4{0, 0, 0, 0};
                    }
#pragma unroll 1
                    for (int ks = 0; ks < th.y; ++ks) {
                        i32x4 a[3];
#pragma unroll
                        for (int q = 0; q < 3; ++q) a[q] = __builtin_bit_cast(i32x4, tt.blk[th.z + tap_dense_block(ks, q, lane)]);
                        u32x4_t g[4];
                        tload(ct, ks, g);
#pragma unroll
                        for (int c = 0; c < 4; ++c) {
                            const i32x4 bq = vb_bop(g, c);
#pragma unroll
                            for (int q = 0; q < 3; ++q)
                                acc[c][q] = __builtin_amdgcn_mfma_i32_16x16x64_i8(a[q], bq, acc[c][q], 0, 0, 0);
                        }
                    }
                    epilogue(ct, [&](int c, int r) { return planes3(acc[c][0][r], acc[c][1][r], acc[c][2][r]); });
                }
            }
        };
        switch (th.y <= IPP_VB_HOIST_MAX ? th.y : 0) {
            case 1: tiles(std::integral_constant<int, 1>{}); break;
#if IPP_VB_HOIST_MAX >= 2
            case 2: tiles(std::integral_constant<int, 2>{}); break;
#endif
#if IPP_VB_HOIST_MAX >= 3
            case 3: tiles(std::integral_constant<int, 3>{}); break;
#endif
#if IPP_VB_HOIST_MAX >= 4
            case 4: tiles(std::integral_constant<int, 4>{}); break;
#endif
            default: tiles(std::integral_constant<int, 0>{}); break;
        }
        __syncthreads();
    }

    const int row_bytes = 3 * p.bg_w;
    if (groups) {
        const int gx0 = p.x >> 4, gx1 = (p.x + p.ov_w + 15) >> 4;
        if ((int)threadIdx.x < gtotal) gload(threadIdx.x, gcur);
        for (int idx = threadIdx.x; idx < gtotal; idx += 256) {
            uint4 gnxt[3];
            if (idx + 256 < gtotal) gload(idx + 256, gnxt);
            const int rr = pow2 ? idx >> lg : idx / G;
            const int gi = gc0 + idx - rr * G;
            uint32_t w[12];
#pragma unroll
            for (int q = 0; q < 3; ++q) {
                w[4 * q] = gcur[q].x;
                w[4 * q + 1] = gcur[q].y;
                w[4 * q + 2] = gcur[q].z;
                w[4 * q + 3] = gcur[q].w;
            }
            const int o = y0 + rr - p.y;
            if (any && o >= oy_lo && o < oy_hi && gi >= gx0 && gi < gx1) {
                const uint4* orw = reinterpret_cast<const uint4*>(orow + rr * os + 16 * (gi - gx0));
                uint32_t ov[16];
#pragma unroll
                for (int q = 0; q < 4; ++q) {
                    const uint4 v4 = orw[q];
                    ov[4 * q] = v4.x;
                    ov[4 * q + 1] = v4.y;
                    ov[4 * q + 2] = v4.z;
                    ov[4 * q + 3] = v4.w;
                }
                blend48(w, ov);
            }
            uint8_t* dp = dsb + (int64_t)rr * p.dst_pitch + 48 * gi;
#pragma unroll
            for (int q = 0; q < 3; ++q) store16<0>(dp + 16 * q, 16, true, w + 4 * q);
#pragma unroll
            for (int q = 0; q < 3; ++q) gcur[q] = gnxt[q];
        }
        return;
    }
    const int chunks = (row_bytes + 15) >> 4;
    const int total = nrows * chunks;
    for (int base = threadIdx.x; base < total; base += 4 * 256) {
        uint32_t w[4][4];
        int rr[4], c0[4], nb[4];
#pragma unroll
        for (int u = 0; u < 4; ++u) {
            const int idx = base + u * 256;
            rr[u] = idx / chunks;
            c0[u] = (idx - rr[u] * chunks) << 4;
            nb[u] = idx < total ? min(16, row_bytes - c0[u]) : 0;
            if (nb[u] > 0) {
                const uint8_t* bp = bg + p.bg_off + (int64_t)(y0 + rr[u]) * p.bg_pitch + c0[u];
                load16(bp, nb[u], nb[u] == 16 && (reinterpret_cast<uintptr_t>(bp) & 15u) == 0, w[u]);
            }
        }
#pragma unroll
        for (int u = 0; u < 4; ++u) {
            if (nb[u] <= 0) continue;
            const int o = y0 + rr[u] - p.y;
            if (any && o >= oy_lo && o < oy_hi && c0[u] + nb[u] > 3 * p.x && c0[u] < 3 * (p.x + p.ov_w)) {
                const uint32_t* orw = orow + rr[u] * os + xo;
                blend16(w[u], c0[u], nb[u], p.x, p.ov_w, [&](int ox) { return orw[ox]; });
            }
            uint8_t* dp = dst + p.dst_off + (int64_t)(y0 + rr[u]) * p.dst_pitch + c0[u];
            store16<0>(dp, nb[u], nb[u] == 16 && (reinterpret_cast<uintptr_t>(dp) & 15u) == 0, w[u]);
        }
    }
}

#if IPP_VB_WPE > 0
#define IPP_VB_ATTR __attribute__((amdgpu_waves_per_eu(IPP_VB_WPE)))
#else
#define IPP_VB_ATTR
#endif
template <bool MAGIC>
__global__ void __launch_bounds__(256) IPP_VB_ATTR
k_pipe_vblend_mfma(const uint8_t* __restrict__ tmp, const uint8_t* __restrict__ bg, uint8_t* __restrict__ dst,
                   const int32_t* __restrict__ coefs, const ipp_pipe_desc* __restrict__ descs, FastDiv tiles_y,
                   int ov_w_max) {
    extern __shared__ __attribute__((aligned(16))) uint32_t orow[];
    const uint32_t b = xcd_remap(blockIdx.x, gridDim.x);
    const int im = (int)fdiv(b, tiles_y);
    const int ty = (int)(b - (uint32_t)im * tiles_y.d);
    vblend_block<MAGIC>(orow, tmp, bg, dst, coefs, descs, im, ty, ov_w_max);
}

template <bool MAGIC>
__global__ void __launch_bounds__(256) IPP_VB_ATTR
k_pipe_vblend_over(const uint8_t* __restrict__ tmp, uint8_t* img, const int32_t* __restrict__ coefs,
                   const ipp_pipe_desc* __restrict__ descs, FastDiv tiles_y, int ov_w_max) {
    extern __shared__ __attribute__((aligned(16))) uint32_t orow[];
    const uint32_t b = xcd_remap(blockIdx.x, gridDim.x);
    const int im = (int)fdiv(b, tiles_y);
    const int ty = (int)(b - (uint32_t)im * tiles_y.d);
    vblend_block<MAGIC, true>(orow, tmp, img, img, coefs, descs, im, ty, ov_w_max);
}

template <int NR, bool ZONES, int CN>
void launch_hpass(int n, int ty, hipStream_t s, const uint8_t* src, uint8_t* tmp, const int32_t* coefs,
                  const ipp_pipe_desc* descs, const ipp_hsv_params& hp, const uint8_t* bg, uint8_t* dst) {
    const int64_t groups = (n + kCopyGroup - 1) / kCopyGroup;
    const uint32_t per_grp = (uint32_t)(kCopyGroup * ty + (bg ? kCopySlabs : 0));
    hipLaunchKernelGGL((k_pipe_hpass2<NR, ZONES, CN>), dim3((uint32_t)(groups * per_grp)), dim3(64 * HP_NW), 0, s,
                       src, tmp, coefs, descs, n, fast_div((uint32_t)ty), fast_div(per_grp), hp, bg, dst);
}

template <int NR>
void launch_hpass_nr(bool zones, int cn, int n, int ty, hipStream_t s, const uint8_t* src, uint8_t* tmp,
                     const int32_t* coefs, const ipp_pipe_desc* descs, const ipp_hsv_params& hp, const uint8_t* bg,
                     uint8_t* dst) {
    if (zones) {
        if (cn == 4) launch_hpass<NR, true, 4>(n, ty, s, src, tmp, coefs, descs, hp, bg, dst);
        else launch_hpass<NR, true, 3>(n, ty, s, src, tmp, coefs, descs, hp, bg, dst);
    } else {
        if (cn == 4) launch_hpass<NR, false, 4>(n, ty, s, src, tmp, coefs, descs, hp, bg, dst);
        else launch_hpass<NR, false, 3>(n, ty, s, src, tmp, coefs, descs, hp, bg, dst);
    }
}

int hpass_entry(const uint8_t* src, uint8_t* tmp, const int32_t* coefs, const ipp_pipe_desc* descs, int32_t n_images,
                int32_t max_out_w, int32_t max_rows, int32_t src_cn, const ipp_hsv_params* hsv, int32_t tap_format,
                const uint8_t* bg, uint8_t* dst, void* stream) {
    if (n_images == 0) return IPP_OK;
    if (!src || !tmp || !coefs || !descs || !hsv || n_images < 0 || max_out_w <= 0 || max_rows <= 0)
        return IPP_E_ARG;
    if (src_cn != 3 && src_cn != 4) return IPP_E_ARG;
    if (tap_format != IPP_TAPS_MFMA) return IPP_E_ARG;
    const int ty = (max_rows + HR - 1) / HR;
    if ((int64_t)(kCopyGroup * ty + kCopySlabs) * ((n_images + kCopyGroup - 1) / kCopyGroup) >= INT32_MAX)
        return IPP_E_ARG;
    hipStream_t s = (hipStream_t)stream;
    bool zones = false;
    for (int k = 0; k < hsv->n_ranges; ++k)
        for (int m = 0; m < 4; ++m) zones |= hsv->r[k].zone[m] != 0;
    const int cn = src_cn, n = n_images;
    const ipp_hsv_range never = ipp_hsv_range{{0, 0, 1}, {180, 255, 0}, {0, 0, 0, 0}};
    switch (hsv->n_ranges) {
        case 1: launch_hpass_nr<1>(zones, cn, n, ty, s, src, tmp, coefs, descs, *hsv, bg, dst); break;
        case 2: launch_hpass_nr<2>(zones, cn, n, ty, s, src, tmp, coefs, descs, *hsv, bg, dst); break;
        case 3: launch_hpass_nr<3>(zones, cn, n, ty, s, src, tmp, coefs, descs, *hsv, bg, dst); break;
        case 4: launch_hpass_nr<4>(zones, cn, n, ty, s, src, tmp, coefs, descs, *hsv, bg, dst); break;
        case 5: case 6: {
            ipp_hsv_params q = *hsv;
            for (int k = q.n_ranges; k < 6; ++k) q.r[k] = never;
            launch_hpass_nr<6>(zones, cn, n, ty, s, src, tmp, coefs, descs, q, bg, dst);
            break;
        }
        default: {
            if (hsv->n_ranges > IPP_MAX_HSV_RANGES) return IPP_E_ARG;
            ipp_hsv_params q = *hsv;
            for (int k = q.n_ranges; k < IPP_MAX_HSV_RANGES; ++k) q.r[k] = never;
            launch_hpass_nr<IPP_MAX_HSV_RANGES>(zones, cn, n, ty, s, src, tmp, coefs, descs, q, bg, dst);
            break;
        }
    }
    IPP_CHECK_LAUNCH();
    return IPP_OK;
}

}

extern "C" int ipp_pipe_hpass_bgcopy(const uint8_t* src, uint8_t* tmp, const int32_t* coefs,
                                     const ipp_pipe_desc* descs, int32_t n_images, int32_t max_out_w,
                                     int32_t max_rows, int32_t src_cn, const ipp_hsv_params* hsv,
                                     int32_t tap_format, const uint8_t* bg, uint8_t* dst, void* stream) {
    if (n_images == 0) return IPP_OK;
    if (!bg || !dst) return IPP_E_ARG;
    return hpass_entry(src, tmp, coefs, descs, n_images, max_out_w, max_rows, src_cn, hsv, tap_format, bg, dst, stream);
}

extern "C" int ipp_pipe_hpass(const uint8_t* src, uint8_t* tmp, const int32_t* coefs, const ipp_pipe_desc* descs,
                              int32_t n_images, int32_t max_out_w, int32_t max_rows, int32_t src_cn,
                              const ipp_hsv_params* hsv, int32_t tap_format, void* stream) {
    return hpass_entry(src, tmp, coefs, descs, n_images, max_out_w, max_rows, src_cn, hsv, tap_format, nullptr,
                       nullptr, stream);
}

extern "C" int ipp_pipe_status(int32_t* status, void* stream) {
    if (!status) return IPP_E_ARG;
    hipStream_t s = (hipStream_t)stream;
    const int32_t zero = 0;
    if (hipMemcpyFromSymbolAsync(status, HIP_SYMBOL(g_pipe_status), sizeof(int32_t), 0, hipMemcpyDeviceToHost, s) !=
            hipSuccess ||
        hipMemcpyToSymbolAsync(HIP_SYMBOL(g_pipe_status), &zero, sizeof(int32_t), 0, hipMemcpyHostToDevice, s) !=
            hipSuccess ||
        hipStreamSynchronize(s) != hipSuccess)
        return IPP_E_LAUNCH;
    return IPP_OK;
}

static int vblend_entry(const uint8_t* tmp, const uint8_t* bg, uint8_t* dst, const int32_t* coefs,
                        const ipp_pipe_desc* descs, int32_t n_images, int32_t bg_w, int32_t bg_h, int32_t max_ov_w,
                        int32_t max_ov_h, int32_t tap_format, void* stream) {
    if (n_images == 0) return IPP_OK;
    if (!tmp || !dst || !coefs || !descs || n_images < 0 || bg_w <= 0 || bg_h <= 0) return IPP_E_ARG;
    if (tap_format != IPP_TAPS_MFMA || max_ov_w <= 0 || max_ov_w > bg_w || max_ov_h <= 0 || max_ov_h > bg_h ||
        max_ov_w > IPP_PIPE_MAX_OV_W)
        return IPP_E_ARG;
    const size_t rows = (size_t)kBandRows * orow_stride(max_ov_w) * sizeof(uint32_t);
    const size_t magic = 256 * sizeof(uint32_t);
    const bool use_magic = rows + magic <= 64 * 1024;
    const int tyb = std::min(paste_max_bands(max_ov_h), (bg_h + kBandRows - 1) / kBandRows);
    const int64_t nb = (int64_t)tyb * n_images;
    if (nb >= INT32_MAX) return IPP_E_ARG;
    hipStream_t st = (hipStream_t)stream;
    const FastDiv ftyb = fast_div((uint32_t)tyb);
    if (!bg) {
        if (use_magic)
            hipLaunchKernelGGL(k_pipe_vblend_over<true>, dim3((uint32_t)nb), dim3(256), rows + magic, st, tmp, dst,
                               coefs, descs, ftyb, max_ov_w);
        else
            hipLaunchKernelGGL(k_pipe_vblend_over<false>, dim3((uint32_t)nb), dim3(256), rows, st, tmp, dst, coefs,
                               descs, ftyb, max_ov_w);
        IPP_CHECK_LAUNCH();
        return IPP_OK;
    }
    if (use_magic)
        hipLaunchKernelGGL(k_pipe_vblend_mfma<true>, dim3((uint32_t)nb), dim3(256), rows + magic, st, tmp, bg, dst,
                           coefs, descs, ftyb, max_ov_w);
    else
        hipLaunchKernelGGL(k_pipe_vblend_mfma<false>, dim3((uint32_t)nb), dim3(256), rows, st, tmp, bg, dst, coefs,
                           descs, ftyb, max_ov_w);
    IPP_CHECK_LAUNCH();
    return IPP_OK;
}

extern "C" int ipp_pipe_vblend_bands(const uint8_t* tmp, const uint8_t* bg, uint8_t* dst, const int32_t* coefs,
                                     const ipp_pipe_desc* descs, int32_t n_images, int32_t bg_w, int32_t bg_h,
                                     int32_t max_ov_w, int32_t max_ov_h, int32_t tap_format, void* stream) {
    if (n_images == 0) return IPP_OK;
    if (!bg) return IPP_E_ARG;
    return vblend_entry(tmp, bg, dst, coefs, descs, n_images, bg_w, bg_h, max_ov_w, max_ov_h, tap_format, stream);
}

extern "C" int ipp_pipe_vblend_over(const uint8_t* tmp, uint8_t* dst, const int32_t* coefs,
                                    const ipp_pipe_desc* descs, int32_t n_images, int32_t bg_w, int32_t bg_h,
                                    int32_t max_ov_w, int32_t max_ov_h, int32_t tap_format, void* stream) {
    return vblend_entry(tmp, nullptr, dst, coefs, descs, n_images, bg_w, bg_h, max_ov_w, max_ov_h, tap_format, stream);
}
```

### image_processor_pipeline_amd/csrc/ipp_pipe_layout.h

```cpp
#pragma once
#include <stdint.h>

#include "ipp.h"

#ifdef __HIPCC__
#define IPP_HD __host__ __device__ __forceinline__
#else
#define IPP_HD inline
#endif

namespace pipe_layout {

constexpr int kTileOut = 16;
constexpr int kTileOutLog2 = 4;
constexpr int kKStepCols = 64;
constexpr int kTapPlanes = 3;
constexpr int kHdrWords = 4;
constexpr int kBiasWords = kTileOut;
constexpr int kKStepBlocks = kTapPlanes * kKStepCols;
constexpr int kKStepBytes = 16 * kKStepBlocks;
constexpr int kCompactMeta = 4;
constexpr int kCompactBlocks = kCompactMeta + kKStepBlocks;
constexpr int kBandRows = 16;
constexpr int kTGroupRows = 4;
constexpr int kTGroupRowsLog2 = 2;
constexpr int kTGroupBytes = 16;
constexpr int kTAlphaByte = 12;
constexpr int kKStepGroups = kKStepCols / kTGroupRows;

IPP_HD constexpr int imin(int a, int b) { return a < b ? a : b; }
IPP_HD constexpr int imax(int a, int b) { return a > b ? a : b; }

IPP_HD constexpr int tap_ntiles(int out_len, int phase) { return (out_len + phase + kTileOut - 1) >> kTileOutLog2; }
IPP_HD constexpr int64_t tap_bias_word(int ntiles) { return kHdrWords * (int64_t)ntiles; }
IPP_HD constexpr int64_t tap_block_word(int ntiles) { return (kHdrWords + kBiasWords) * (int64_t)ntiles; }
IPP_HD constexpr int tap_dense_block(int ks, int plane, int lane) { return (ks * kTapPlanes + plane) * kKStepCols + lane; }
IPP_HD constexpr int tap_compact_block(int plane, int i) { return kCompactMeta + plane * kKStepCols + i; }
IPP_HD constexpr int64_t tap_tile_block(int t, int nkb) { return (int64_t)t * nkb * kKStepBlocks; }
IPP_HD constexpr int64_t tap_axis_words(int64_t ntiles, int nkb) {
    return (kHdrWords + kBiasWords) * ntiles + ntiles * nkb * (kKStepBytes / 4);
}

IPP_HD constexpr int tap_phase(int y) { return y & (kBandRows - 1); }
IPP_HD constexpr int band_tap_tile(int y0, int y, int phase) { return (y0 - y + phase) >> 4; }
IPP_HD void paste_bands(const ipp_paste_desc& p, int& vb0, int& vb1) {
    vb0 = (p.y >> 4) << 4;
    vb1 = imin(p.bg_h, ((p.y + p.ov_h + 15) >> 4) << 4);
    vb1 = imax(vb1, vb0);
}
IPP_HD constexpr int paste_max_bands(int max_ov_h) { return (max_ov_h + 15 + kBandRows - 1) / kBandRows; }

template <typename Aligned>
IPP_HD bool band_cols_split(const ipp_paste_desc& p, int& gx0, int& gx1, Aligned aligned) {
    const int rb = 3 * p.bg_w;
    gx0 = imax(p.x, 0) >> 4;
    gx1 = imin((p.x + p.ov_w + 15) >> 4, p.bg_w >> 4);
    const int64_t lr = 3 * (p.bg_w >> 4);
    return (p.bg_w & 15) == 0 && p.bg_pitch == rb && p.dst_pitch == rb && gx0 < gx1 &&
           (int64_t)p.bg_h * lr * lr < (1ll << 32) && aligned();
}

IPP_HD constexpr int t_row_group(int row) { return row >> kTGroupRowsLog2; }
IPP_HD constexpr int t_pitch_vecs(int pitch_bytes) { return pitch_bytes >> 4; }
IPP_HD constexpr int64_t t_groups(int rows, int nkb_v) {
    return (((int64_t)(rows + 15) / 16) * 16 + kKStepCols * nkb_v + 16) / kTGroupRows;
}

static_assert(tap_block_word(1) == 20 && tap_bias_word(1) == 4, "blocks begin at word 20·T, bias at 4·T (ipp.h)");
static_assert((1 << kTileOutLog2) == kTileOut && (1 << kTGroupRowsLog2) == kTGroupRows, "the shifts");
static_assert(kKStepBytes == 3072, "3072 bytes per K step (ipp.h, ipp_plan_mfma_tile)");
static_assert(tap_tile_block(1, 1) == 192 && tap_tile_block(5, 3) == 5 * 3 * 192, "tile t's blocks at t·nkb·192 (ipp.h)");
static_assert(tap_compact_block(1, 5) == kCompactMeta + tap_dense_block(0, 1, 5), "compact blocks: the meta, then K step 0's lane map");
static_assert(tap_axis_words(1, 1) == 20 + 768 && tap_ntiles(16, 0) == 1 && tap_ntiles(16, 1) == 2, "axis size");
static_assert(kKStepGroups == 16 && kTAlphaByte == 3 * 4 && kTGroupBytes == 4 * kTGroupRows, "T group");
static_assert(paste_max_bands(1) == 1 && paste_max_bands(2) == 2 && paste_max_bands(17) == 2 && paste_max_bands(18) == 3,
              "bands of an overlay");
static_assert(kBandRows * 4 * (IPP_PIPE_MAX_OV_W + 32) == 64 * 1024, "IPP_PIPE_MAX_OV_W is the band's LDS limit");

#ifdef __HIPCC__
typedef int32_t i32x4 __attribute__((ext_vector_type(4)));
typedef uint32_t u32x4_t __attribute__((ext_vector_type(4)));

struct TapTiles {
    const int4* hdr;
    const int32_t* bias;
    const uint4* blk;
};
__device__ __forceinline__ TapTiles tap_tiles(const int32_t* coefs, int64_t coef_off, int ntiles) {
    return TapTiles{reinterpret_cast<const int4*>(coefs + coef_off), coefs + coef_off + tap_bias_word(ntiles),
                    reinterpret_cast<const uint4*>(coefs + coef_off + tap_block_word(ntiles))};
}

typedef uint4 TGroup;
static_assert(sizeof(TGroup) == kTGroupBytes, "one 16-B vector per T group");
template <typename V>
__device__ __forceinline__ const V* t_group(const V* base, int pitch, int group, int x) {
    static_assert(sizeof(V) == kTGroupBytes, "a pointer to whole groups");
    return base + x + (int64_t)group * pitch;
}
#endif

}
```

### image_processor_pipeline_amd/fused.py

```python
from __future__ import annotations

import math
import os
import random
import time
from dataclasses import dataclass, field
from typing import List, Optional, Sequence, Tuple

import numpy as np
import torch

from . import _native as N
from . import geometry as G
from .device import SYM_FLIP, _stream, _to_dev
from .device import check_alpha_min as _check_alpha_min
from .labels_fmt import (instance_ids, scene_contour_capacity, scene_instance_masks, scene_labels,
                         scene_map_pitch, scene_seg_labels, seg_label, simplify_tolerance, xyxy2xywhn, yolo_label,
                         yolo_labels)

ALL_SYMS = ("o", "h", "v", "hv")
H_RING_COLUMNS = 512


@dataclass
class PipeConfig:
    margins: Tuple[float, float, float, float] = (64, 64, 64, 64)
    angle_min: float = 1.0
    angle_max: float = 359.0
    sym_pool: Tuple[str, ...] = ALL_SYMS
    hsv_ranges: list = field(default_factory=lambda: list(G.REFERENCE_HSV_RANGES))
    zones: Optional[list] = None
    use_gimp_scale: bool = False
    scale_min: float = 0.15
    scale_max: float = 0.30


@dataclass
class ItemParams:
    angle: float
    sym: str
    bg_index: int
    ratio: float
    x: int = 0
    y: int = 0


@dataclass
class PipePlan:
    descs: np.ndarray
    axes: np.ndarray
    coef_words: int
    hsv: np.ndarray
    items: np.ndarray
    sym_pool: Tuple[str, ...]
    tmp_bytes: int
    max_out_w: int
    max_rows: int
    bg_w: int
    bg_h: int
    algo_bytes_hpass: int = 0
    algo_bytes_vblend: int = 0
    tap_format: int = 1
    max_ov_w: int = 1
    max_ov_h: int = 1
    algo_bytes_hpass_bgcopy: int = 0
    algo_bytes_vblend_bands: int = 0
    copy_read_bytes: int = 0

    @property
    def params(self) -> List[ItemParams]:
        it = self.items
        return [ItemParams(float(a), self.sym_pool[s], int(b), float(r), int(x), int(y))
                for a, s, b, r, x, y in zip(it["angle"], it["sym"], it["bg_index"], it["ratio"], it["x"], it["y"])]

    @property
    def order(self) -> np.ndarray:
        return np.argsort(self.items["bg_index"], kind="stable")

    @property
    def cut_dims(self) -> List[Tuple[int, int]]:
        return list(zip(self.items["cut_h"].tolist(), self.items["cut_w"].tolist()))

    @property
    def ov_dims(self) -> List[Tuple[int, int]]:
        return list(zip(self.items["ov_h"].tolist(), self.items["ov_w"].tolist()))


def draw_params(n_global: int, stop: int, src_hw: Tuple[int, int], bg_hw: Tuple[int, int], n_bg: int,
                cfg: PipeConfig, seed: int):
    H, W = src_hw
    bh, bw = bg_hw
    rng = random.Random(seed)
    pool = list(cfg.sym_pool)
    angles = [rng.uniform(cfg.angle_min, cfg.angle_max) for _ in range(n_global)]
    syms = [rng.sample(pool, 1)[0] for _ in range(n_global)]
    order = list(range(n_bg))
    rng.shuffle(order)
    t, b, l, r = G.crop_margins(H, W, cfg.margins)
    wc, hc = W - l - r, H - t - b
    per_item = []
    for gi in range(stop):
        ratio = rng.uniform(cfg.scale_min, cfg.scale_max)
        plan, box, (nw_, nh_) = item_geometry(wc, hc, angles[gi], ratio, bw, bh, gi)
        x = rng.randint(0, bw - nw_)
        y = rng.randint(0, bh - nh_)
        per_item.append((ratio, x, y, plan, box, (nw_, nh_)))
    return angles, syms, order, per_item


def item_geometry(wc: int, hc: int, angle: float, ratio: float, bw: int, bh: int, gi: int = 0):
    plan = G.rotation_plan(wc, hc, angle)
    bb = G.rotated_bbox(wc, hc, plan)
    if bb is not None and bb[2] > bb[0] and bb[3] > bb[1]:
        box = (bb[0], bb[1], bb[2] - bb[0], bb[3] - bb[1])
    else:
        box = (0, 0, plan.nw, plan.nh)
    nw_, nh_ = G.overlay_size(box[2], box[3], bw, bh, ratio)
    if nw_ <= 0 or nh_ <= 0:
        raise ValueError(f"item {gi}: degenerate overlay size {nw_}x{nh_}")
    return plan, box, (nw_, nh_)


def shard_range(n_global: int, rank: int, world: int) -> Tuple[int, int]:
    if world <= 0 or not 0 <= rank < world:
        raise ValueError(f"bad rank/world {rank}/{world}")
    q, rem = divmod(n_global, world)
    start = rank * q + min(rank, rem)
    return start, start + q + (1 if rank < rem else 0)


def plan_threads() -> int:
    try:
        n = int(os.environ.get("OMP_NUM_THREADS", "0"))
    except ValueError:
        n = 0
    if n <= 0:
        n = len(os.sched_getaffinity(0)) if hasattr(os, "sched_getaffinity") else (os.cpu_count() or 1)
    return max(1, min(n, 32))


_PLAN_ERRORS = {
    1: (NotImplementedError, "rotation canvas beyond Pillow's 16.16 fixed-point range (>32767 px)"),
    2: (NotImplementedError, "non-affine ScaleAffine table"),
    3: (ValueError, "degenerate overlay size"),
    4: (ValueError, "parameters do not fit the background (position, background index or symmetry)"),
    5: (ValueError, "LANCZOS downscale needs a tap window wider than the fused H pass's 512-column LDS ring; "
                    "use the plugin path"),
    6: (ValueError, "empty range for randrange() (overlay larger than the background)"),
}


def plan_pipe(src_hw: Tuple[int, int], n: int, bg_hw: Tuple[int, int], n_bg: int, cfg: PipeConfig,
              seed: int = 0, src_pitch: Optional[int] = None, item_range: Optional[Tuple[int, int]] = None,
              n_global: Optional[int] = None, params: Optional[Sequence[ItemParams]] = None,
              n_threads: int = 0) -> PipePlan:
    H, W = src_hw
    bh, bw = bg_hw
    start, stop = item_range if item_range is not None else (0, n)
    if stop - start != n or start < 0 or n <= 0:
        raise ValueError(f"item_range {item_range} does not hold {n} items")
    n_global = stop if n_global is None else n_global
    if n_global < stop:
        raise ValueError(f"n_global {n_global} < item_range stop {stop}")
    t, b, l, r = G.crop_margins(H, W, cfg.margins)
    items = np.zeros(n, N.PIPE_ITEM)
    c = np.zeros((), N.PIPE_PLAN_CFG)
    pool = tuple(cfg.sym_pool)
    given = params
    if given is None and not (isinstance(seed, int) and abs(seed) < 1 << 64):
        angles, syms, order, drawn = draw_params(n_global, stop, src_hw, bg_hw, n_bg, cfg, seed)
        given = [ItemParams(angles[g], syms[g], order[g % n_bg], drawn[g][0], drawn[g][1], drawn[g][2])
                 for g in range(start, stop)]
    if given is not None:
        if len(given) != n:
            raise ValueError(f"{len(given)} ItemParams for {n} items")
        pool = ALL_SYMS
        for i, it in enumerate(given):
            if it.sym not in SYM_FLIP:
                raise ValueError(f"item {start + i}: parameters {it} do not fit a {bw}x{bh} background")
        items["angle"] = [it.angle for it in given]
        items["ratio"] = [it.ratio for it in given]
        items["sym"] = [ALL_SYMS.index(it.sym) for it in given]
        items["bg_index"] = [it.bg_index for it in given]
        items["x"] = [it.x for it in given]
        items["y"] = [it.y for it in given]
        c["given"] = 1
    else:
        if not 1 <= len(pool) <= 4 or any(p not in SYM_FLIP for p in pool):
            raise ValueError(f"symmetry pool {pool}: 1 to 4 of {ALL_SYMS}")
        c["seed"] = abs(seed)
    c["src_h"], c["src_w"], c["src_pitch"] = H, W, src_pitch or 0
    c["crop_t"], c["crop_b"], c["crop_l"], c["crop_r"] = t, b, l, r
    c["bg_h"], c["bg_w"], c["n_bg"] = bh, bw, n_bg
    c["n_sym"] = len(pool)
    c["sym_flip"][:len(pool)] = [SYM_FLIP[p] for p in pool]
    c["n_global"], c["start"], c["stop"] = n_global, start, stop
    c["angle_min"], c["angle_max"] = cfg.angle_min, cfg.angle_max
    c["scale_min"], c["scale_max"] = cfg.scale_min, cfg.scale_max
    c["n_threads"] = n_threads or plan_threads()
    c["ring_cols"] = H_RING_COLUMNS
    descs = np.zeros(n, N.PIPE_DESC)
    axes = np.zeros(2 * n, N.TAP_AXIS)
    tot = np.zeros(N.IPP_PLAN_TOTALS, np.int64)
    lib = N.load()
    rc = lib.ipp_plan_pipe_batch(N.np_ptr(c), N.np_ptr(items), N.np_ptr(descs), N.np_ptr(axes), N.np_ptr(tot))
    if rc == N.IPP_E_RANGE and int(tot[N.PT["err_code"]]) in _PLAN_ERRORS:
        exc, msg = _PLAN_ERRORS[int(tot[N.PT["err_code"]])]
        raise exc(f"item {int(tot[N.PT['err_item']])}: {msg}")
    N.check(rc, "ipp_plan_pipe_batch")
    T = {k: int(tot[v]) for k, v in N.PT.items()}
    if T["max_ov_w"] > N.IPP_PIPE_MAX_OV_W:
        raise ValueError(f"overlay width {T['max_ov_w']} px exceeds the fused pipe's limit of "
                         f"{N.IPP_PIPE_MAX_OV_W} px (ipp_pipe_vblend_bands); use the file-mode plugins")
    hsv = G.hsv_params(cfg.hsv_ranges, cfg.zones, cfg.use_gimp_scale, bgr=False)
    return PipePlan(descs, axes, T["coef_words"], hsv, items, pool, T["tmp_bytes"], T["max_out_w"], T["max_rows"],
                    bw, bh, T["algo_h"], T["algo_v"], N.IPP_TAPS_MFMA, T["max_ov_w"], T["max_ov_h"],
                    T["algo_h"] + T["copy_bytes"], T["algo_v"] - T["copy_bytes"], T["copy_reads"])


def plan_taps(plan: PipePlan, device, stream=None) -> Tuple[torch.Tensor, int]:
    lib = N.load()
    device = torch.device(device)
    coefs = torch.empty(plan.coef_words + 4096, dtype=torch.int32, device=device)
    nb = lib.ipp_pipe_taps_scratch_bytes(len(plan.axes))
    scratch = torch.empty(int(nb), dtype=torch.uint8, device=device)
    stats = np.zeros(2, np.int64)
    N.check(lib.ipp_pipe_plan_taps(N.np_ptr(plan.axes), len(plan.axes), coefs.data_ptr(), scratch.data_ptr(),
                                   N.np_ptr(stats), stream if stream is not None else _stream(device)),
            "ipp_pipe_plan_taps")
    if stats[1]:
        raise N.NativeError(f"ipp_pipe_plan_taps: device status {int(stats[1])} (tile beyond its K-step bound)")
    return coefs, int(stats[0])


def overlap_bounds(n: int, parts: int, ratio: float = 1.0, group: int = N.IPP_PIPE_COPY_GROUP) -> List[int]:
    if n < 0 or parts < 1 or ratio <= 0:
        raise ValueError(f"overlap_bounds: n={n} parts={parts} ratio={ratio}")
    groups = (n + group - 1) // group
    w = [ratio ** k for k in range(parts)]
    cum = [sum(w[:k]) / sum(w) for k in range(parts + 1)]
    b = [min(n, group * int(round(groups * c))) for c in cum]
    b[-1] = n
    return b


def _launch_hpass_bgcopy(lib, plan: PipePlan, src: int, tmp: int, coefs: int, descs: int, n: int, bgs: int, out: int,
                         stream: int) -> None:
    N.check(lib.ipp_pipe_hpass_bgcopy(src, tmp, coefs, descs, n, plan.max_out_w, plan.max_rows, 3, N.np_ptr(plan.hsv),
                                      plan.tap_format, bgs, out, stream), "ipp_pipe_hpass_bgcopy")


def _launch_vblend_bands(lib, plan: PipePlan, tmp: int, bgs: int, out: int, coefs: int, descs: int, n: int,
                         stream: int) -> None:
    N.check(lib.ipp_pipe_vblend_bands(tmp, bgs, out, coefs, descs, n, plan.bg_w, plan.bg_h, plan.max_ov_w,
                                      plan.max_ov_h, plan.tap_format, stream), "ipp_pipe_vblend_bands")


class _Runner:

    def __init__(self, plan, device):
        pipe = getattr(plan, "pipe", plan)
        self.plan = plan
        self.device = torch.device(device)
        self.descs = _to_dev(plan.descs, self.device)
        self.coefs, self.host_tiles = plan_taps(pipe, self.device)
        self.tmp = torch.empty(pipe.tmp_bytes, dtype=torch.uint8, device=self.device)
        self.lib = N.load()
        self._hpass_done = False

    def _dptr(self, d0: int) -> int:
        return self.descs.data_ptr() + d0 * self.plan.descs.itemsize

    def _check_tensors(self, caller: str, src: torch.Tensor, bgs: torch.Tensor, out: torch.Tensor) -> None:
        who = f"{type(self).__name__}.{caller}"
        for t, name in ((src, "src"), (bgs, "bgs"), (out, "out")):
            if not (t.is_cuda and t.dtype == torch.uint8 and t.is_contiguous()):
                raise N.NativeUnavailable(f"{who}: {name} must be a contiguous uint8 ROCm tensor")

    def status(self) -> int:
        st = np.zeros(1, np.int32)
        N.check(self.lib.ipp_pipe_status(N.np_ptr(st), _stream(self.device)), "ipp_pipe_status")
        return int(st[0])


class PipeRunner(_Runner):

    def hpass_bgcopy(self, src: torch.Tensor, bgs: torch.Tensor, out: torch.Tensor, items=None) -> None:
        p = self.plan
        i0, n = items if items is not None else (0, len(p.descs))
        _launch_hpass_bgcopy(self.lib, p, src.data_ptr(), self.tmp.data_ptr(), self.coefs.data_ptr(),
                             self._dptr(i0), n, bgs.data_ptr(), out.data_ptr(), _stream(self.device))
        self._hpass_done = True

    def overlay_bboxes(self, alpha_min: int = 1, items=None) -> np.ndarray:
        alpha_min = _check_alpha_min(alpha_min)
        i0, n = items if items is not None else (0, len(self.plan.descs))
        if n <= 0:
            return np.zeros((0, 4), np.int32)
        return self._bboxes_by_item(self._launch_bboxes(alpha_min, i0, n), i0, n)

    def _launch_bboxes(self, alpha_min: int, i0: int, n: int) -> torch.Tensor:
        alpha_min = _check_alpha_min(alpha_min)
        if not self._hpass_done:
            raise N.NativeError("PipeRunner.overlay_bboxes: no H launch (hpass_bgcopy) has run on this runner")
        p = self.plan
        bbox = torch.empty(4 * max(n, 0), dtype=torch.int32, device=self.device)
        N.check(self.lib.ipp_pipe_overlay_bbox(self.tmp.data_ptr(), self.coefs.data_ptr(), self._dptr(i0), n,
                                               p.max_ov_w, p.max_ov_h, alpha_min, p.tap_format, bbox.data_ptr(),
                                               _stream(self.device)), "ipp_pipe_overlay_bbox")
        return bbox

    def _bboxes_by_item(self, bbox: torch.Tensor, i0: int, n: int) -> np.ndarray:
        by_desc = bbox.cpu().numpy().reshape(-1, 4)
        rank = np.argsort(np.argsort(self.plan.order[i0:i0 + n], kind="stable"), kind="stable")
        out = np.empty_like(by_desc)
        out[rank] = by_desc
        return out

    def vblend_bands(self, bgs: torch.Tensor, out: torch.Tensor, items=None) -> None:
        p = self.plan
        i0, n = items if items is not None else (0, len(p.descs))
        _launch_vblend_bands(self.lib, p, self.tmp.data_ptr(), bgs.data_ptr(), out.data_ptr(), self.coefs.data_ptr(),
                             self._dptr(i0), n, _stream(self.device))

    def run_overlapped(self, src: torch.Tensor, bgs: torch.Tensor, out: torch.Tensor, parts: int,
                       ratio: float = 1.0) -> None:
        self._check_tensors("run_overlapped", src, bgs, out)
        bounds = overlap_bounds(len(self.plan.descs), parts, ratio)
        main = torch.cuda.current_stream(self.device)
        if getattr(self, "_vstream", None) is None:
            self._vstream = torch.cuda.Stream(self.device)
            self._events = []
        side = self._vstream
        while len(self._events) < parts:
            self._events.append(torch.cuda.Event())
        side.wait_stream(main)
        for k in range(parts):
            i0, i1 = bounds[k], bounds[k + 1]
            if i1 <= i0:
                continue
            self.hpass_bgcopy(src, bgs, out, items=(i0, i1 - i0))
            ev = self._events[k]
            ev.record(main)
            side.wait_event(ev)
            with torch.cuda.stream(side):
                self.vblend_bands(bgs, out, items=(i0, i1 - i0))
        main.wait_stream(side)

    @property
    def split(self) -> bool:
        return self.plan.tap_format == N.IPP_TAPS_MFMA

    def run(self, src: torch.Tensor, bgs: torch.Tensor, out: torch.Tensor) -> torch.Tensor:
        self._check_tensors("run", src, bgs, out)
        if not self.split:
            raise N.NativeError(f"PipeRunner.run: tap format {self.plan.tap_format} (the pipe takes IPP_TAPS_MFMA)")
        self.hpass_bgcopy(src, bgs, out)
        self.vblend_bands(bgs, out)
        return out

    def run_labelled(self, src: torch.Tensor, bgs: torch.Tensor, out: torch.Tensor, tight: bool = True,
                     alpha_min: int = 1, class_id: int = 0) -> Tuple[torch.Tensor, List[Optional[str]]]:
        self._check_tensors("run_labelled", src, bgs, out)
        if not self.split:
            raise N.NativeError(f"PipeRunner.run_labelled: tap format {self.plan.tap_format} "
                                "(the pipe takes IPP_TAPS_MFMA)")
        if tight:
            alpha_min = _check_alpha_min(alpha_min)
        self.hpass_bgcopy(src, bgs, out)
        n = len(self.plan.descs)
        bbox = self._launch_bboxes(alpha_min, 0, n) if tight else None
        self.vblend_bands(bgs, out)
        return out, yolo_labels(self.plan, class_id, self._bboxes_by_item(bbox, 0, n) if tight else None)


class PipeStream:

    def __init__(self, device, plan_fn, slots: int = 3, priority: bool = True, lookahead: int = 2):
        self.device = torch.device(device)
        self.plan_fn = plan_fn
        self.lib = N.load()
        self.lookahead = max(1, int(lookahead))
        slots = max(slots, self.lookahead + 1)
        self.main = torch.cuda.Stream(self.device, priority=-1) if priority else None
        self.slots = [{"done": torch.cuda.Event(), "bufs": {}, "side": torch.cuda.Stream(self.device)}
                      for _ in range(max(2, slots))]
        self.timing: List[Tuple[float, float, int]] = []
        self.events: List[Tuple[torch.cuda.Event, torch.cuda.Event]] = []

    def _buf(self, slot, name: str, nbytes: int) -> torch.Tensor:
        b = slot["bufs"].get(name)
        if b is None or b.numel() < nbytes:
            slot["bufs"][name] = None
            b = torch.empty(max(int(nbytes), 256), dtype=torch.uint8, device=self.device)
            slot["bufs"][name] = b
        return b

    def _prepare(self, k: int, slot):
        t0 = time.perf_counter()
        plan = self.plan_fn(k)
        t1 = time.perf_counter()
        slot["done"].synchronize()
        bufs = {"descs": self._buf(slot, "descs", plan.descs.nbytes),
                "coefs": self._buf(slot, "coefs", 4 * (plan.coef_words + 4096)),
                "tmp": self._buf(slot, "tmp", plan.tmp_bytes),
                "scratch": self._buf(slot, "scratch", self.lib.ipp_pipe_taps_scratch_bytes(len(plan.axes)))}
        stats = np.zeros(2, np.int64)
        side = slot["side"]
        with torch.cuda.stream(side):
            bufs["descs"][:plan.descs.nbytes].copy_(torch.from_numpy(plan.descs.view(np.uint8)))
            N.check(self.lib.ipp_pipe_plan_taps(N.np_ptr(plan.axes), len(plan.axes), bufs["coefs"].data_ptr(),
                                                bufs["scratch"].data_ptr(), N.np_ptr(stats),
                                                side.cuda_stream), "ipp_pipe_plan_taps")
        if stats[1]:
            raise N.NativeError(f"ipp_pipe_plan_taps: device status {int(stats[1])}")
        t2 = time.perf_counter()
        return plan, bufs, ((t1 - t0) * 1e3, (t2 - t1) * 1e3, int(stats[0]))

    def run(self, n_batches: int, src: torch.Tensor, bgs: torch.Tensor, out: torch.Tensor, mark=None,
            record: bool = False) -> None:
        from concurrent.futures import ThreadPoolExecutor
        main = self.main if self.main is not None else torch.cuda.current_stream(self.device)
        if self.main is not None:
            self.main.wait_stream(torch.cuda.current_stream(self.device))
        L, ns = self.lookahead, len(self.slots)
        with ThreadPoolExecutor(L) as ex:
            futs = {j: ex.submit(self._prepare, j, self.slots[j % ns]) for j in range(min(L, n_batches))}
            for k in range(n_batches):
                plan, b, tm = futs.pop(k).result()
                if mark is not None and k == mark.at:
                    mark()
                slot = self.slots[k % ns]
                if k + L < n_batches:
                    futs[k + L] = ex.submit(self._prepare, k + L, self.slots[(k + L) % ns])
                ev = (torch.cuda.Event(enable_timing=True), torch.cuda.Event(enable_timing=True)) if record else None
                if ev:
                    ev[0].record(main)
                _launch_hpass_bgcopy(self.lib, plan, src.data_ptr(), b["tmp"].data_ptr(), b["coefs"].data_ptr(),
                                     b["descs"].data_ptr(), len(plan.descs), bgs.data_ptr(), out.data_ptr(),
                                     main.cuda_stream)
                _launch_vblend_bands(self.lib, plan, b["tmp"].data_ptr(), bgs.data_ptr(), out.data_ptr(),
                                     b["coefs"].data_ptr(), b["descs"].data_ptr(), len(plan.descs), main.cuda_stream)
                if ev:
                    ev[1].record(main)
                    self.events.append(ev)
                slot["done"].record(main)
                self.timing.append(tm)
        if self.main is not None:
            torch.cuda.current_stream(self.device).wait_stream(self.main)


_SCENE_NAMES = ("draw_scene_params", "ScenePlan", "plan_scenes", "SIMPLIFY_MAX_SIDE", "SceneRunner")


def __getattr__(name: str):
    if name not in _SCENE_NAMES:
        raise AttributeError(f"module {__name__!r} has no attribute {name!r}")
    from . import scenes
    return getattr(scenes, name)


def __dir__():
    return sorted({*globals(), *_SCENE_NAMES})
```

### include/ipp.h

```cpp
#ifndef IPP_H
#define IPP_H

#include <stdint.h>

#ifdef __cplusplus
extern "C" {
#endif

#define IPP_OK 0
#define IPP_E_ARG (-1)
#define IPP_E_LAUNCH (-2)
#define IPP_E_RANGE (-3)

#define IPP_MAX_HSV_RANGES 16

typedef struct ipp_gather_desc {
    int64_t src_off;
    int64_t dst_off;
    int32_t src_pitch;
    int32_t src_cn;
    int32_t src_w, src_h;
    int32_t in_x0, in_y0, in_w, in_h;
    int32_t a0, a1, a2, a3, a4, a5;
    int32_t out_w, out_h;
    int32_t off_x, off_y;
    int32_t flip;
    int32_t dst_pitch;
    int64_t base_off;
    uint32_t lim;
    int32_t b[6];
    int32_t prepared;
} ipp_gather_desc;

int ipp_gather_prepare(ipp_gather_desc* descs, int32_t n);

int ipp_rotate_flip_nearest(const uint8_t* src, uint8_t* dst,
                            const ipp_gather_desc* descs, int32_t n_images,
                            int32_t max_out_w, int32_t max_out_h, void* stream);

typedef struct ipp_affine_desc {
    int64_t src_off, dst_off;
    int32_t src_pitch, src_cn;
    int32_t in_x0, in_y0, in_w, in_h;
    int32_t out_w, out_h, dst_pitch;
    int32_t flip;
    double m[6];
} ipp_affine_desc;

int ipp_rotate_bilinear(const uint8_t* src, uint8_t* dst, const ipp_affine_desc* descs,
                        int32_t n_images, int32_t max_out_w, int32_t max_out_h, void* stream);

typedef struct ipp_copy_desc {
    int64_t src_off, dst_off;
    int32_t src_pitch, dst_pitch;
    int32_t x0, y0, w, h;
    int32_t cn;
    int32_t flip;
} ipp_copy_desc;

int ipp_copy_window(const uint8_t* src, uint8_t* dst, const ipp_copy_desc* descs,
                    int32_t n_images, int32_t max_w, int32_t max_h, void* stream);

int ipp_crop_to_bbox(const uint8_t* src, uint8_t* dst, const ipp_copy_desc* descs,
                     const int32_t* bbox, int32_t n_images, int32_t max_w, int32_t max_h,
                     int32_t cn, void* stream);

typedef struct ipp_hsv_range {
    int32_t lo[3], hi[3];
    int32_t zone[4];
} ipp_hsv_range;

typedef struct ipp_hsv_params {
    int32_t n_ranges;
    int32_t bgr;
    ipp_hsv_range r[IPP_MAX_HSV_RANGES];
} ipp_hsv_params;

typedef struct ipp_image_desc {
    int64_t off;
    int32_t w, h, pitch;
    int32_t cn;
} ipp_image_desc;

int ipp_hsv_mask(const uint8_t* src, const ipp_image_desc* src_descs,
                 uint8_t* dst, const ipp_image_desc* dst_descs, int32_t n_images,
                 int32_t max_w, int32_t max_h, const ipp_hsv_params* params, void* stream);

typedef struct ipp_resample_desc {
    int64_t src_off, dst_off;
    int32_t src_pitch, dst_pitch;
    int32_t in_len;
    int32_t out_len;
    int32_t lines;
    int32_t line0;
    int32_t ksize;
    int32_t pad_;
    int64_t coef_off;
} ipp_resample_desc;

#define IPP_RS_PREMULTIPLY 1
#define IPP_RS_UNPREMULTIPLY 2

int ipp_lanczos_h(const uint8_t* src, uint8_t* dst, const int32_t* coefs,
                  const ipp_resample_desc* descs, int32_t n_images,
                  int32_t max_out, int32_t max_lines, int32_t flags, void* stream);
int ipp_lanczos_v(const uint8_t* src, uint8_t* dst, const int32_t* coefs,
                  const ipp_resample_desc* descs, int32_t n_images,
                  int32_t max_out, int32_t max_lines, int32_t flags, void* stream);

typedef struct ipp_paste_desc {
    int64_t bg_off, ov_off, dst_off;
    int32_t bg_w, bg_h, bg_pitch, dst_pitch;
    int32_t ov_w, ov_h, ov_pitch;
    int32_t x, y;
    int32_t pad_;
} ipp_paste_desc;

int ipp_paste_blend(const uint8_t* bg, const uint8_t* ov, uint8_t* dst,
                    const ipp_paste_desc* descs, int32_t n_images,
                    int32_t bg_w, int32_t bg_h, void* stream);

typedef struct ipp_pipe_desc {
    ipp_gather_desc g;
    ipp_resample_desc h;
    ipp_resample_desc v;
    ipp_paste_desc p;
} ipp_pipe_desc;

#define IPP_TAPS_MFMA 1

int ipp_pipe_hpass_bgcopy(const uint8_t* src, uint8_t* tmp, const int32_t* coefs,
                          const ipp_pipe_desc* descs, int32_t n_images,
                          int32_t max_out_w, int32_t max_rows, int32_t src_cn,
                          const ipp_hsv_params* hsv, int32_t tap_format,
                          const uint8_t* bg, uint8_t* dst, void* stream);
int ipp_pipe_vblend_bands(const uint8_t* tmp, const uint8_t* bg, uint8_t* dst,
                          const int32_t* coefs, const ipp_pipe_desc* descs, int32_t n_images,
                          int32_t bg_w, int32_t bg_h, int32_t max_ov_w, int32_t max_ov_h,
                          int32_t tap_format, void* stream);

int ipp_pipe_status(int32_t* status, void* stream);

int ipp_pipe_overlay_bbox(const uint8_t* tmp, const int32_t* coefs, const ipp_pipe_desc* descs,
                          int32_t n_images, int32_t max_ov_w, int32_t max_ov_h,
                          int32_t alpha_min, int32_t tap_format, int32_t* bbox, void* stream);

int ipp_pipe_hpass(const uint8_t* src, uint8_t* tmp, const int32_t* coefs,
                   const ipp_pipe_desc* descs, int32_t n_images, int32_t max_out_w,
                   int32_t max_rows, int32_t src_cn, const ipp_hsv_params* hsv,
                   int32_t tap_format, void* stream);
int ipp_pipe_vblend_over(const uint8_t* tmp, uint8_t* dst, const int32_t* coefs,
                         const ipp_pipe_desc* descs, int32_t n_images, int32_t bg_w, int32_t bg_h,
                         int32_t max_ov_w, int32_t max_ov_h, int32_t tap_format, void* stream);
int64_t ipp_pipe_scene_scratch_bytes(int32_t n_images, int32_t n_scenes, int32_t per_scene,
                                     int32_t max_ov_w, int32_t max_ov_h);
int ipp_pipe_scene_boxes(const uint8_t* tmp, const int32_t* coefs, const ipp_pipe_desc* descs,
                         const int32_t* scene_layer, int32_t n_images, int32_t n_scenes,
                         int32_t per_scene, int32_t max_ov_w, int32_t max_ov_h, int32_t alpha_min,
                         int32_t cover_min, int32_t tap_format, uint8_t* scratch, int32_t* out,
                         void* stream);
#define IPP_SCENE_MAP_MAX_LAYERS 8
int ipp_pipe_scene_map(const uint8_t* tmp, const int32_t* coefs, const ipp_pipe_desc* descs,
                       const int32_t* scene_layer, int32_t n_images, int32_t n_scenes, int32_t per_scene,
                       int32_t bg_w, int32_t bg_h, int32_t max_ov_w, int32_t max_ov_h,
                       int32_t alpha_min, int32_t cover_min, int32_t tap_format,
                       uint8_t* scratch, int32_t* rows ,
                       uint8_t* map, int64_t map_pitch, void* stream);

#define IPP_CONTOUR_HDR 8
int64_t ipp_scene_contours_scratch_bytes(int32_t n_images, int32_t max_edges);
int ipp_scene_contours(const uint8_t* map, int64_t map_pitch, int32_t bg_w, int32_t bg_h,
                       const int32_t* rows, const int32_t* scene_layer, int32_t n_images,
                       int32_t n_scenes, int32_t per_scene, int32_t max_edges,
                       uint8_t* scratch, int32_t* hdr, void* stream);
int ipp_scene_contours_pack(const uint8_t* scratch, const int32_t* hdr, const int64_t* offsets,
                            int32_t n_images, int32_t max_edges, int32_t* verts, void* stream);

#define IPP_SIMPLIFY_LDS_VERTS 2048
#define IPP_SIMPLIFY_THREADS 256
int64_t ipp_polygons_simplify_scratch_bytes(int32_t n_images, int64_t total_vertices);
int ipp_polygons_simplify(const int32_t* verts, const int64_t* offsets, const int32_t* hdr, int32_t n_images,
                          int64_t total_vertices, int32_t bg_w, int32_t bg_h, int32_t eps_q, uint8_t* scratch,
                          int32_t* counts, void* stream);
int ipp_polygons_simplify_pack(const int32_t* verts, const int64_t* offsets, const int32_t* hdr,
                               const uint8_t* scratch, const int32_t* counts, const int64_t* out_offsets,
                               int32_t n_images, int32_t* out, void* stream);

typedef struct ipp_ccl_work {
    int64_t mask_off, edge_off, p_off, a_off, ent_off;
    int64_t ent_cap;
    int64_t tile_off;
    int64_t img_off;
} ipp_ccl_work;

int64_t ipp_ccl_scratch_layout(int32_t w, int32_t h, ipp_ccl_work* work);

int ipp_ccl_keep_largest(uint8_t* img, const ipp_image_desc* descs, int32_t n_images,
                         int32_t max_w, int32_t max_h, const ipp_ccl_work* works,
                         uint8_t* scratch, int64_t max_ent, int32_t* counts, int64_t* stats,
                         int32_t* bbox, void* stream);

int ipp_video_keep_largest(const uint8_t* frames, const ipp_image_desc* descs, int32_t n_images,
                           int32_t max_w, int32_t max_h, const ipp_hsv_params* hsv,
                           const ipp_ccl_work* works, uint8_t* scratch, int64_t max_ent,
                           int32_t* counts, int64_t* stats, int32_t* bbox, uint8_t* out,
                           const ipp_image_desc* out_descs, void* stream);

int ipp_alpha_bbox(const uint8_t* img, const ipp_image_desc* descs, int32_t n_images,
                   int32_t max_w, int32_t max_h, int32_t* bbox, void* stream);
int ipp_alpha_bbox_min(const uint8_t* img, const ipp_image_desc* descs, int32_t n_images,
                       int32_t max_w, int32_t max_h, int32_t alpha_min, int32_t* bbox,
                       void* stream);

int64_t ipp_plan_lanczos(int32_t in_size, double in0, double in1, int32_t out_size,
                         int32_t* out, int64_t out_capacity);
int ipp_plan_lanczos_batch(int32_t n, const int32_t* in_sizes, const int32_t* out_sizes,
                           const int64_t* offsets, int32_t* out, int64_t out_capacity,
                           int32_t n_threads);
int ipp_plan_pipe_axes(int32_t n, const int32_t* in_sizes, const int32_t* out_sizes,
                       const int32_t* identity, const int32_t* shift_first,
                       const int32_t* transposed, const int64_t* offsets, int32_t* out,
                       int32_t* first_last, int32_t n_threads);
int64_t ipp_plan_mfma_size(int32_t in_size, int32_t out_size, int32_t ksize);
int32_t ipp_plan_mfma_nk_bound(int32_t in_size, int32_t out_size, int32_t ksize);
int ipp_plan_mfma_from_taps(int32_t in_size, int32_t out_size, int32_t ksize,
                            const int32_t* std_taps, int32_t shift, int32_t phase, int32_t* out);
int32_t ipp_plan_lanczos_ksize(double in0, double in1, int32_t out_size);

int ipp_plan_opaque_bbox(int32_t in_w, int32_t in_h, const int32_t a[6],
                         int32_t nw, int32_t nh, int32_t bbox[4]);

typedef struct ipp_pipe_plan_cfg {
    int32_t src_h, src_w, src_pitch;
    int32_t crop_t, crop_b, crop_l, crop_r;
    int32_t bg_h, bg_w, n_bg;
    int32_t n_sym, sym_flip[4];
    int32_t n_global, start, stop;
    int32_t given;
    int32_t n_threads;
    int32_t ring_cols;
    int32_t pad_;
    uint64_t seed;
    double angle_min, angle_max, scale_min, scale_max;
} ipp_pipe_plan_cfg;

typedef struct ipp_pipe_item {
    double angle, ratio;
    int32_t sym, bg_index, x, y;
    int32_t rot_w, rot_h;
    int32_t cut_x, cut_y, cut_w, cut_h;
    int32_t ov_w, ov_h;
} ipp_pipe_item;

typedef struct ipp_tap_axis {
    int32_t in_size, out_size;
    int32_t identity;
    int32_t shift;
    int32_t phase;
    int32_t nkb;
    int32_t compact;
    int32_t n_tiles;
    int64_t coef_off;
} ipp_tap_axis;

#define IPP_PT_COEF_WORDS 0
#define IPP_PT_TMP_BYTES 1
#define IPP_PT_MAX_OUT_W 2
#define IPP_PT_MAX_ROWS 3
#define IPP_PT_MAX_OV_W 4
#define IPP_PT_MAX_OV_H 5
#define IPP_PT_ALGO_H 6
#define IPP_PT_ALGO_V 7
#define IPP_PT_COPY_BYTES 8
#define IPP_PT_MAX_TILES 9
#define IPP_PT_ERR_ITEM 10
#define IPP_PT_ERR_CODE 11
#define IPP_PT_COPY_READS 12
#define IPP_PLAN_TOTALS 16

#define IPP_PIPE_COPY_GROUP 8
#define IPP_PIPE_MAX_OV_W 992

int ipp_plan_pipe_batch(const ipp_pipe_plan_cfg* cfg, ipp_pipe_item* items, ipp_pipe_desc* descs,
                        ipp_tap_axis* axes, int64_t* totals);

int64_t ipp_pipe_taps_scratch_bytes(int32_t n_axes);
int ipp_pipe_plan_taps(const ipp_tap_axis* axes, int32_t n_axes, int32_t* coefs, void* scratch,
                       int64_t* stats, void* stream);
int ipp_pipe_plan_taps_cap(const ipp_tap_axis* axes, int32_t n_axes, int32_t* coefs, void* scratch,
                           int64_t* stats, int64_t pack_cap, void* stream);
int ipp_plan_mfma_tile(const ipp_tap_axis* axis, int32_t t, int32_t hdr[4], int32_t bias[16],
                       uint8_t* blocks, int64_t blocks_cap);
int ipp_plan_opaque_bbox_fast(int32_t in_w, int32_t in_h, const int32_t a[6],
                              int32_t nw, int32_t nh, int32_t bbox[4]);
double ipp_plan_py_hypot(double x, double y);
int ipp_plan_rotation(int32_t w, int32_t h, double angle, int32_t out[8]);
int ipp_plan_py_random(uint64_t seed, int32_t n, double* out);

#define IPP_ENH_BLUR 1
#define IPP_ENH_LUT 2

typedef struct ipp_enhance_desc {
    int64_t src_off, dst_off;
    int32_t w, h, src_pitch, dst_pitch;
    float f_brightness, f_contrast, f_color;
    int32_t flags;
    int32_t box_r;
    uint32_t box_ww, box_fw;
    int32_t pad_;
    int64_t lut_off;
} ipp_enhance_desc;

int ipp_enhance_lsum(const uint8_t* src, const ipp_enhance_desc* descs, int32_t n_images,
                     int64_t max_pixels, uint64_t* sums, void* stream);
int ipp_enhance_color(const uint8_t* src, uint8_t* dst, const ipp_enhance_desc* descs,
                      int32_t n_images, int64_t max_pixels, const uint64_t* sums,
                      const uint8_t* luts, void* stream);
int ipp_box_pass(const uint8_t* src, uint8_t* dst, const ipp_enhance_desc* descs, int32_t n_images,
                 int64_t max_pixels, const int64_t* offs, int32_t axis, const uint8_t* luts,
                 int32_t final_dst, void* stream);

int ipp_stream_copy(const uint8_t* src, uint8_t* dst, int64_t nbytes, void* stream);

const char* ipp_version(void);

#ifdef __cplusplus
}
#endif
#endif
```

Baseline: 458,800.

## Pass per-band transparent-column trim metadata from hpass to vblend and bbox

The horizontal pass now records, for each 16-row band, the span of column tiles that hold non-transparent content. It no longer writes the constant fill into the trimmed tiles of tmp. The vertical blend and overlay bbox kernels read this trim table and substitute the constant 0x80 pattern in registers for tiles outside the span, skipping those tmp loads. This cuts HBM writes in hpass and reads in vblend, at the cost of a small trim buffer and per-K-step branch logic in the MFMA loops.

```diff
diff --git a/image_processor_pipeline_amd/_native.py b/image_processor_pipeline_amd/_native.py
--- a/image_processor_pipeline_amd/_native.py
+++ b/image_processor_pipeline_amd/_native.py
@@ -131,6 +131,9 @@
     "ipp_alpha_bbox": (_I, [_P, _P, _I, _I, _I, _P, _P]),
     "ipp_alpha_bbox_min": (_I, [_P, _P, _I, _I, _I, _I, _P, _P]),
     "ipp_pipe_overlay_bbox": (_I, [_P, _P, _P, _I, _I, _I, _I, _I, _P, _P]),
+    "ipp_pipe_hpass_bgcopy_trim": (_I, [_P, _P, _P, _P, _I, _I, _I, _I, _P, _I, _P, _P, _P, _P]),
+    "ipp_pipe_vblend_bands_trim": (_I, [_P, _P, _P, _P, _P, _I, _I, _I, _I, _I, _I, _P, _I, _P]),
+    "ipp_pipe_overlay_bbox_trim": (_I, [_P, _P, _P, _I, _I, _I, _I, _I, _P, _P, _I, _P]),
     "ipp_pipe_hpass": (_I, [_P, _P, _P, _P, _I, _I, _I, _I, _P, _I, _P]),
     "ipp_pipe_vblend_over": (_I, [_P, _P, _P, _P, _I, _I, _I, _I, _I, _I, _P]),
     "ipp_pipe_scene_scratch_bytes": (_L, [_I, _I, _I, _I, _I]),
diff --git a/image_processor_pipeline_amd/csrc/ipp_label.hip b/image_processor_pipeline_amd/csrc/ipp_label.hip
--- a/image_processor_pipeline_amd/csrc/ipp_label.hip
+++ b/image_processor_pipeline_amd/csrc/ipp_label.hip
@@ -40,7 +40,7 @@
 template <typename Sink>
 __device__ __forceinline__ void overlay_alpha_band(const uint8_t* __restrict__ tmp, const int32_t* __restrict__ coefs,
                                                    const ipp_pipe_desc* __restrict__ descs, int im, int ty,
-                                                   Sink sink) {
+                                                   const uint16_t* __restrict__ trim, Sink sink) {
     const ipp_paste_desc p = descs[im].p;
     int vb0, vb1;
     paste_bands(p, vb0, vb1);
@@ -67,6 +67,7 @@
 #pragma unroll
     for (int r = 0; r < 4; ++r) rb[r] = tt.bias[kBiasWords * t + 4 * (lane >> 4) + r];
     const int gbase = t_row_group(th.x + 16 * (lane >> 4));
+    const int hbands = trim_bands(descs[im].h.lines);
     const uint8_t* abase = tmp + v.src_off + gbase * gstride * kTGroupBytes + kTAlphaByte;
 
     for (int ct = wave; ct < ctiles; ct += 4) {
@@ -79,10 +80,17 @@
         acc[2] = i32x4{0, 0, 0, 0};
 #pragma unroll 1
         for (int ks = 0; ks < th.y; ++ks) {
-            i32x4 bq;
-#pragma unroll
-            for (int j = 0; j < 4; ++j)
-                bq[j] = *reinterpret_cast<const int32_t*>(aq + (kKStepGroups * ks + j) * gstride * kTGroupBytes);
+            uint32_t e = kTrimNone;
+            if (trim) {
+                const int hb = trim_v_band(th.x, ks, lane);
+                e = hb < hbands ? (uint32_t)trim[hb] : kTrimAll;
+            }
+            i32x4 bq = i32x4{(int32_t)0x80808080u, (int32_t)0x80808080u, (int32_t)0x80808080u, (int32_t)0x80808080u};
+            if (!trim_const(e, ct)) {
+#pragma unroll
+                for (int j = 0; j < 4; ++j)
+                    bq[j] = *reinterpret_cast<const int32_t*>(aq + (kKStepGroups * ks + j) * gstride * kTGroupBytes);
+            }
 #pragma unroll
             for (int q = 0; q < 3; ++q) {
                 const i32x4 a = __builtin_bit_cast(i32x4, tt.blk[th.z + tap_dense_block(ks, q, lane)]);
@@ -102,12 +110,13 @@
 __global__ void __launch_bounds__(256)
 k_pipe_overlay_bbox(const uint8_t* __restrict__ tmp, const int32_t* __restrict__ coefs,
                     const ipp_pipe_desc* __restrict__ descs, FastDiv tiles_y, int alpha_min,
-                    int32_t* __restrict__ bbox) {
+                    int32_t* __restrict__ bbox, const uint16_t* __restrict__ trim, int trim_stride) {
     const uint32_t b = xcd_remap(blockIdx.x, gridDim.x);
     const int im = (int)fdiv(b, tiles_y);
     const int ty = (int)(b - (uint32_t)im * tiles_y.d);
     int xmin = INT32_MAX, ymin = INT32_MAX, xmax = -1, ymax = -1;
-    overlay_alpha_band(tmp, coefs, descs, im, ty, [&](int x, int o, int a) {
+    const uint16_t* trow = trim ? trim + (int64_t)im * trim_stride : nullptr;
+    overlay_alpha_band(tmp, coefs, descs, im, ty, trow, [&](int x, int o, int a) {
         if (a >= alpha_min) {
             xmin = min(xmin, x);
             xmax = max(xmax, x);
@@ -179,7 +188,7 @@
     if (descs[im].p.ov_w > max_ov_w || descs[im].p.ov_h > max_ov_h) return;
     const int64_t pitch = scene_pitch(max_ov_w);
     uint8_t* plane = planes + (int64_t)im * max_ov_h * pitch;
-    overlay_alpha_band(tmp, coefs, descs, im, ty,
+    overlay_alpha_band(tmp, coefs, descs, im, ty, nullptr,
                        [&](int x, int o, int a) { plane[(int64_t)o * pitch + x] = (uint8_t)a; });
 }
 
@@ -359,11 +368,13 @@
 
 }
 
-extern "C" int ipp_pipe_overlay_bbox(const uint8_t* tmp, const int32_t* coefs, const ipp_pipe_desc* descs,
-                                     int32_t n_images, int32_t max_ov_w, int32_t max_ov_h, int32_t alpha_min,
-                                     int32_t tap_format, int32_t* bbox, void* stream) {
+extern "C" int ipp_pipe_overlay_bbox_trim(const uint8_t* tmp, const int32_t* coefs, const ipp_pipe_desc* descs,
+                                          int32_t n_images, int32_t max_ov_w, int32_t max_ov_h, int32_t alpha_min,
+                                          int32_t tap_format, int32_t* bbox, const uint16_t* trim, int32_t max_rows,
+                                          void* stream) {
     if (alpha_min < 1 || alpha_min > 255 || tap_format != IPP_TAPS_MFMA) return IPP_E_ARG;
     if (!tmp || !coefs || !descs || !bbox || n_images < 0 || max_ov_w <= 0 || max_ov_h <= 0) return IPP_E_ARG;
+    if (trim && max_rows <= 0) return IPP_E_ARG;
     if (n_images == 0) return IPP_OK;
     const int tyb = paste_max_bands(max_ov_h);
     const int64_t nb = (int64_t)tyb * n_images;
@@ -372,10 +383,17 @@
     const int ib = (n_images + 255) / 256;
     hipLaunchKernelGGL(k_label_bbox_init, dim3(ib), dim3(256), 0, s, bbox, n_images);
     hipLaunchKernelGGL(k_pipe_overlay_bbox, dim3((uint32_t)nb), dim3(256), 0, s, tmp, coefs, descs,
-                       fast_div((uint32_t)tyb), alpha_min, bbox);
+                       fast_div((uint32_t)tyb), alpha_min, bbox, trim, trim ? trim_bands(max_rows) : 0);
     hipLaunchKernelGGL(k_label_bbox_finish, dim3(ib), dim3(256), 0, s, bbox, n_images);
     IPP_CHECK_LAUNCH();
     return IPP_OK;
+}
+
+extern "C" int ipp_pipe_overlay_bbox(const uint8_t* tmp, const int32_t* coefs, const ipp_pipe_desc* descs,
+                                     int32_t n_images, int32_t max_ov_w, int32_t max_ov_h, int32_t alpha_min,
+                                     int32_t tap_format, int32_t* bbox, void* stream) {
+    return ipp_pipe_overlay_bbox_trim(tmp, coefs, descs, n_images, max_ov_w, max_ov_h, alpha_min, tap_format, bbox,
+                                      nullptr, 0, stream);
 }
 
 extern "C" int ipp_alpha_bbox_min(const uint8_t* img, const ipp_image_desc* descs, int32_t n_images,
diff --git a/image_processor_pipeline_amd/csrc/ipp_pipe.hip b/image_processor_pipeline_amd/csrc/ipp_pipe.hip
--- a/image_processor_pipeline_amd/csrc/ipp_pipe.hip
+++ b/image_processor_pipeline_amd/csrc/ipp_pipe.hip
@@ -539,7 +539,7 @@
 __device__ __forceinline__ void hpass_block(Hpass2Lds<NR>& L, const uint8_t* __restrict__ src,
                                             uint8_t* __restrict__ tmp, const int32_t* __restrict__ coefs,
                                             const ipp_pipe_desc* __restrict__ descs, int im, int tb,
-                                            const ipp_hsv_params& hp) {
+                                            const ipp_hsv_params& hp, uint16_t* __restrict__ trim) {
     const ipp_gather_desc g = descs[im].g;
     const ipp_resample_desc h = descs[im].h;
     const int row0 = tb * HR;
@@ -630,7 +630,7 @@
             const uint64_t km = __builtin_amdgcn_ballot_w64(keep);
             s_lo = km ? __builtin_ctzll(km) : 0;
             s_hi = km ? 64 - __builtin_clzll(km) : 0;
-            const int ntrim = s_lo + ntiles - s_hi;
+            const int ntrim = trim ? 0 : s_lo + ntiles - s_hi;
             for (int i = wave; i < ntrim; i += HP_NW) {
                 const int t = i < s_lo ? i : i - s_lo + s_hi;
                 const int xo = 16 * t + (lane & 15);
@@ -641,9 +641,10 @@
                     store16<2>(reinterpret_cast<uint8_t*>(dst), kTGroupBytes, true, w);
                 }
             }
-            if (s_lo >= s_hi) return;
-        }
-    }
+        }
+    }
+    if (trim && threadIdx.x == 0) trim[tb] = (uint16_t)trim_entry(s_lo, s_hi);
+    if (s_lo >= s_hi) return;
 
     const int nrows = min(HR, h.lines - row0);
     if (fast)
@@ -656,7 +657,7 @@
 __global__ void __launch_bounds__(64 * HP_NW) __attribute__((amdgpu_waves_per_eu(ZONES ? 3 : 4)))
 k_pipe_hpass2(const uint8_t* __restrict__ src, uint8_t* __restrict__ tmp, const int32_t* __restrict__ coefs,
               const ipp_pipe_desc* __restrict__ descs, int n, FastDiv tiles_y, FastDiv per_grp, ipp_hsv_params hp,
-              const uint8_t* __restrict__ bg, uint8_t* __restrict__ dst) {
+              const uint8_t* __restrict__ bg, uint8_t* __restrict__ dst, uint16_t* __restrict__ trim) {
     __shared__ Hpass2Lds<NR> L;
     const uint32_t b = xcd_remap(blockIdx.x, gridDim.x);
     const int ty = (int)tiles_y.d;
@@ -669,7 +670,7 @@
     const int j = (int)fdiv((uint32_t)t, tiles_y);
     const int im = grp * kCopyGroup + j;
     if (im >= n) return;
-    hpass_block<NR, ZONES, CN>(L, src, tmp, coefs, descs, im, t - j * ty, hp);
+    hpass_block<NR, ZONES, CN>(L, src, tmp, coefs, descs, im, t - j * ty, hp, trim ? trim + (int64_t)im * ty : nullptr);
 }
 
 #ifndef IPP_VB_DB
@@ -766,7 +767,8 @@
 __device__ __forceinline__ void vblend_block(uint32_t* __restrict__ orow, const uint8_t* __restrict__ tmp,
                                              typename VbPtr<INPLACE>::bg_t bg, typename VbPtr<INPLACE>::dst_t dst,
                                              const int32_t* __restrict__ coefs,
-                                             const ipp_pipe_desc* __restrict__ descs, int im, int ty, int ov_w_max) {
+                                             const ipp_pipe_desc* __restrict__ descs, int im, int ty, int ov_w_max,
+                                             const uint16_t* __restrict__ trim) {
     const ipp_paste_desc p = vb_paste_desc(descs[im].p, INPLACE);
     int y0 = ty * kBandRows;
     {
@@ -825,11 +827,22 @@
         for (int r = 0; r < 4; ++r) rb[r] = tt.bias[kBiasWords * t + 4 * (lane >> 4) + r];
         const u32x4_t* tbase = reinterpret_cast<const u32x4_t*>(tmp + v.src_off);
         const int gbase = t_row_group(th.x + 16 * (lane >> 4));
-        auto tload = [&](int ct, int ks, u32x4_t (&g)[4]) {
-            const int xs = min(16 * ct + x_l, p.ov_w - 1);
-            const u32x4_t* tq = t_group(tbase, gstride, gbase + kKStepGroups * ks, xs);
-#pragma unroll
-            for (int j = 0; j < 4; ++j) g[j] = tq[j * gstride];
+        const int hbands = trim_bands(descs[im].h.lines);
+        auto tentry = [&](int ks) -> uint32_t {
+            if (!trim) return kTrimNone;
+            const int hb = trim_v_band(th.x, ks, lane);
+            return hb < hbands ? (uint32_t)trim[hb] : kTrimAll;
+        };
+        auto tload = [&](int ct, int ks, uint32_t e, u32x4_t (&g)[4]) {
+            if (trim_const(e, ct)) {
+#pragma unroll
+                for (int j = 0; j < 4; ++j) g[j] = u32x4_t{0x80808080u, 0x80808080u, 0x80808080u, 0x80808080u};
+            } else {
+                const int xs = min(16 * ct + x_l, p.ov_w - 1);
+                const u32x4_t* tq = t_group(tbase, gstride, gbase + kKStepGroups * ks, xs);
+#pragma unroll
+                for (int j = 0; j < 4; ++j) g[j] = tq[j * gstride];
+            }
         };
         auto epilogue = [&](int ct, auto s) {
             const int x = 16 * ct + x_l;
@@ -854,6 +867,11 @@
 #pragma unroll
                     for (int q = 0; q < 3; ++q)
                         ta[ks][q] = __builtin_bit_cast(i32x4, tt.blk[th.z + tap_dense_block(ks, q, lane)]);
+                static_assert(NK <= 4, "four 16-bit trim entries in 64 bits");
+                uint64_t tpk = 0;
+#pragma unroll
+                for (int ks = 0; ks < NK; ++ks) tpk |= (uint64_t)tentry(ks) << (16 * ks);
+                auto te = [&](int ks) { return (uint32_t)(tpk >> (16 * ks)) & 0xFFFFu; };
                 auto transpose = [&](const u32x4_t (&g)[NK][4], i32x4 (&bq)[NK][4]) {
 #pragma unroll
                     for (int ks = 0; ks < NK; ++ks)
@@ -866,14 +884,14 @@
                     int ct = wave;
                     if (ct < ctiles) {
 #pragma unroll
-                        for (int ks = 0; ks < NK; ++ks) tload(ct, ks, gn[ks]);
+                        for (int ks = 0; ks < NK; ++ks) tload(ct, ks, te(ks), gn[ks]);
                         transpose(gn, bc);
                     }
                     for (; ct < ctiles; ct += 4) {
                         const bool more = ct + 4 < ctiles;
                         if (more) {
 #pragma unroll
-                            for (int ks = 0; ks < NK; ++ks) tload(ct + 4, ks, gn[ks]);
+                            for (int ks = 0; ks < NK; ++ks) tload(ct + 4, ks, te(ks), gn[ks]);
                         }
                         i32x4 acc[4];
                         vb_mfma_tile<NK>(ta, bc, rb, acc);
@@ -884,7 +902,7 @@
                     for (int ct = wave; ct < ctiles; ct += 4) {
                         u32x4_t g[NK][4];
 #pragma unroll
-                        for (int ks = 0; ks < NK; ++ks) tload(ct, ks, g[ks]);
+                        for (int ks = 0; ks < NK; ++ks) tload(ct, ks, te(ks), g[ks]);
                         i32x4 bq[NK][4];
                         transpose(g, bq);
                         i32x4 acc[4];
@@ -907,7 +925,7 @@
 #pragma unroll
                         for (int q = 0; q < 3; ++q) a[q] = __builtin_bit_cast(i32x4, tt.blk[th.z + tap_dense_block(ks, q, lane)]);
                         u32x4_t g[4];
-                        tload(ct, ks, g);
+                        tload(ct, ks, tentry(ks), g);
 #pragma unroll
                         for (int c = 0; c < 4; ++c) {
                             const i32x4 bq = vb_bop(g, c);
@@ -1014,12 +1032,13 @@
 __global__ void __launch_bounds__(256) IPP_VB_ATTR
 k_pipe_vblend_mfma(const uint8_t* __restrict__ tmp, const uint8_t* __restrict__ bg, uint8_t* __restrict__ dst,
                    const int32_t* __restrict__ coefs, const ipp_pipe_desc* __restrict__ descs, FastDiv tiles_y,
-                   int ov_w_max) {
+                   int ov_w_max, const uint16_t* __restrict__ trim, int trim_stride) {
     extern __shared__ __attribute__((aligned(16))) uint32_t orow[];
     const uint32_t b = xcd_remap(blockIdx.x, gridDim.x);
     const int im = (int)fdiv(b, tiles_y);
     const int ty = (int)(b - (uint32_t)im * tiles_y.d);
-    vblend_block<MAGIC>(orow, tmp, bg, dst, coefs, descs, im, ty, ov_w_max);
+    vblend_block<MAGIC>(orow, tmp, bg, dst, coefs, descs, im, ty, ov_w_max,
+                        trim ? trim + (int64_t)im * trim_stride : nullptr);
 }
 
 template <bool MAGIC>
@@ -1030,40 +1049,42 @@
     const uint32_t b = xcd_remap(blockIdx.x, gridDim.x);
     const int im = (int)fdiv(b, tiles_y);
     const int ty = (int)(b - (uint32_t)im * tiles_y.d);
-    vblend_block<MAGIC, true>(orow, tmp, img, img, coefs, descs, im, ty, ov_w_max);
+    vblend_block<MAGIC, true>(orow, tmp, img, img, coefs, descs, im, ty, ov_w_max, nullptr);
 }
 
 template <int NR, bool ZONES, int CN>
 void launch_hpass(int n, int ty, hipStream_t s, const uint8_t* src, uint8_t* tmp, const int32_t* coefs,
-                  const ipp_pipe_desc* descs, const ipp_hsv_params& hp, const uint8_t* bg, uint8_t* dst) {
+                  const ipp_pipe_desc* descs, const ipp_hsv_params& hp, const uint8_t* bg, uint8_t* dst,
+                  uint16_t* trim) {
     const int64_t groups = (n + kCopyGroup - 1) / kCopyGroup;
     const uint32_t per_grp = (uint32_t)(kCopyGroup * ty + (bg ? kCopySlabs : 0));
     hipLaunchKernelGGL((k_pipe_hpass2<NR, ZONES, CN>), dim3((uint32_t)(groups * per_grp)), dim3(64 * HP_NW), 0, s,
-                       src, tmp, coefs, descs, n, fast_div((uint32_t)ty), fast_div(per_grp), hp, bg, dst);
+                       src, tmp, coefs, descs, n, fast_div((uint32_t)ty), fast_div(per_grp), hp, bg, dst, trim);
 }
 
 template <int NR>
 void launch_hpass_nr(bool zones, int cn, int n, int ty, hipStream_t s, const uint8_t* src, uint8_t* tmp,
                      const int32_t* coefs, const ipp_pipe_desc* descs, const ipp_hsv_params& hp, const uint8_t* bg,
-                     uint8_t* dst) {
+                     uint8_t* dst, uint16_t* trim) {
     if (zones) {
-        if (cn == 4) launch_hpass<NR, true, 4>(n, ty, s, src, tmp, coefs, descs, hp, bg, dst);
-        else launch_hpass<NR, true, 3>(n, ty, s, src, tmp, coefs, descs, hp, bg, dst);
+        if (cn == 4) launch_hpass<NR, true, 4>(n, ty, s, src, tmp, coefs, descs, hp, bg, dst, trim);
+        else launch_hpass<NR, true, 3>(n, ty, s, src, tmp, coefs, descs, hp, bg, dst, trim);
     } else {
-        if (cn == 4) launch_hpass<NR, false, 4>(n, ty, s, src, tmp, coefs, descs, hp, bg, dst);
-        else launch_hpass<NR, false, 3>(n, ty, s, src, tmp, coefs, descs, hp, bg, dst);
+        if (cn == 4) launch_hpass<NR, false, 4>(n, ty, s, src, tmp, coefs, descs, hp, bg, dst, trim);
+        else launch_hpass<NR, false, 3>(n, ty, s, src, tmp, coefs, descs, hp, bg, dst, trim);
     }
 }
 
 int hpass_entry(const uint8_t* src, uint8_t* tmp, const int32_t* coefs, const ipp_pipe_desc* descs, int32_t n_images,
                 int32_t max_out_w, int32_t max_rows, int32_t src_cn, const ipp_hsv_params* hsv, int32_t tap_format,
-                const uint8_t* bg, uint8_t* dst, void* stream) {
+                const uint8_t* bg, uint8_t* dst, uint16_t* trim, void* stream) {
     if (n_images == 0) return IPP_OK;
     if (!src || !tmp || !coefs || !descs || !hsv || n_images < 0 || max_out_w <= 0 || max_rows <= 0)
         return IPP_E_ARG;
     if (src_cn != 3 && src_cn != 4) return IPP_E_ARG;
     if (tap_format != IPP_TAPS_MFMA) return IPP_E_ARG;
     const int ty = (max_rows + HR - 1) / HR;
+    static_assert(HR == kBandRows, "an H band is a trim table entry (trim_bands)");
     if ((int64_t)(kCopyGroup * ty + kCopySlabs) * ((n_images + kCopyGroup - 1) / kCopyGroup) >= INT32_MAX)
         return IPP_E_ARG;
     hipStream_t s = (hipStream_t)stream;
@@ -1073,21 +1094,21 @@
     const int cn = src_cn, n = n_images;
     const ipp_hsv_range never = ipp_hsv_range{{0, 0, 1}, {180, 255, 0}, {0, 0, 0, 0}};
     switch (hsv->n_ranges) {
-        case 1: launch_hpass_nr<1>(zones, cn, n, ty, s, src, tmp, coefs, descs, *hsv, bg, dst); break;
-        case 2: launch_hpass_nr<2>(zones, cn, n, ty, s, src, tmp, coefs, descs, *hsv, bg, dst); break;
-        case 3: launch_hpass_nr<3>(zones, cn, n, ty, s, src, tmp, coefs, descs, *hsv, bg, dst); break;
-        case 4: launch_hpass_nr<4>(zones, cn, n, ty, s, src, tmp, coefs, descs, *hsv, bg, dst); break;
+        case 1: launch_hpass_nr<1>(zones, cn, n, ty, s, src, tmp, coefs, descs, *hsv, bg, dst, trim); break;
+        case 2: launch_hpass_nr<2>(zones, cn, n, ty, s, src, tmp, coefs, descs, *hsv, bg, dst, trim); break;
+        case 3: launch_hpass_nr<3>(zones, cn, n, ty, s, src, tmp, coefs, descs, *hsv, bg, dst, trim); break;
+        case 4: launch_hpass_nr<4>(zones, cn, n, ty, s, src, tmp, coefs, descs, *hsv, bg, dst, trim); break;
         case 5: case 6: {
             ipp_hsv_params q = *hsv;
             for (int k = q.n_ranges; k < 6; ++k) q.r[k] = never;
-            launch_hpass_nr<6>(zones, cn, n, ty, s, src, tmp, coefs, descs, q, bg, dst);
+            launch_hpass_nr<6>(zones, cn, n, ty, s, src, tmp, coefs, descs, q, bg, dst, trim);
             break;
         }
         default: {
             if (hsv->n_ranges > IPP_MAX_HSV_RANGES) return IPP_E_ARG;
             ipp_hsv_params q = *hsv;
             for (int k = q.n_ranges; k < IPP_MAX_HSV_RANGES; ++k) q.r[k] = never;
-            launch_hpass_nr<IPP_MAX_HSV_RANGES>(zones, cn, n, ty, s, src, tmp, coefs, descs, q, bg, dst);
+            launch_hpass_nr<IPP_MAX_HSV_RANGES>(zones, cn, n, ty, s, src, tmp, coefs, descs, q, bg, dst, trim);
             break;
         }
     }
@@ -1103,14 +1124,26 @@
                                      int32_t tap_format, const uint8_t* bg, uint8_t* dst, void* stream) {
     if (n_images == 0) return IPP_OK;
     if (!bg || !dst) return IPP_E_ARG;
-    return hpass_entry(src, tmp, coefs, descs, n_images, max_out_w, max_rows, src_cn, hsv, tap_format, bg, dst, stream);
+    return hpass_entry(src, tmp, coefs, descs, n_images, max_out_w, max_rows, src_cn, hsv, tap_format, bg, dst, nullptr,
+                       stream);
+}
+
+extern "C" int ipp_pipe_hpass_bgcopy_trim(const uint8_t* src, uint8_t* tmp, const int32_t* coefs,
+                                          const ipp_pipe_desc* descs, int32_t n_images, int32_t max_out_w,
+                                          int32_t max_rows, int32_t src_cn, const ipp_hsv_params* hsv,
+                                          int32_t tap_format, const uint8_t* bg, uint8_t* dst, uint16_t* trim,
+                                          void* stream) {
+    if (n_images == 0) return IPP_OK;
+    if (!bg || !dst) return IPP_E_ARG;
+    return hpass_entry(src, tmp, coefs, descs, n_images, max_out_w, max_rows, src_cn, hsv, tap_format, bg, dst, trim,
+                       stream);
 }
 
 extern "C" int ipp_pipe_hpass(const uint8_t* src, uint8_t* tmp, const int32_t* coefs, const ipp_pipe_desc* descs,
                               int32_t n_images, int32_t max_out_w, int32_t max_rows, int32_t src_cn,
                               const ipp_hsv_params* hsv, int32_t tap_format, void* stream) {
     return hpass_entry(src, tmp, coefs, descs, n_images, max_out_w, max_rows, src_cn, hsv, tap_format, nullptr,
-                       nullptr, stream);
+                       nullptr, nullptr, stream);
 }
 
 extern "C" int ipp_pipe_status(int32_t* status, void* stream) {
@@ -1128,9 +1161,10 @@
 
 static int vblend_entry(const uint8_t* tmp, const uint8_t* bg, uint8_t* dst, const int32_t* coefs,
                         const ipp_pipe_desc* descs, int32_t n_images, int32_t bg_w, int32_t bg_h, int32_t max_ov_w,
-                        int32_t max_ov_h, int32_t tap_format, void* stream) {
+                        int32_t max_ov_h, int32_t tap_format, const uint16_t* trim, int32_t max_rows, void* stream) {
     if (n_images == 0) return IPP_OK;
     if (!tmp || !dst || !coefs || !descs || n_images < 0 || bg_w <= 0 || bg_h <= 0) return IPP_E_ARG;
+    if (trim && (max_rows <= 0 || !bg)) return IPP_E_ARG;
     if (tap_format != IPP_TAPS_MFMA || max_ov_w <= 0 || max_ov_w > bg_w || max_ov_h <= 0 || max_ov_h > bg_h ||
         max_ov_w > IPP_PIPE_MAX_OV_W)
         return IPP_E_ARG;
@@ -1152,12 +1186,13 @@
         IPP_CHECK_LAUNCH();
         return IPP_OK;
     }
+    const int tstride = trim ? trim_bands(max_rows) : 0;
     if (use_magic)
         hipLaunchKernelGGL(k_pipe_vblend_mfma<true>, dim3((uint32_t)nb), dim3(256), rows + magic, st, tmp, bg, dst,
-                           coefs, descs, ftyb, max_ov_w);
+                           coefs, descs, ftyb, max_ov_w, trim, tstride);
     else
         hipLaunchKernelGGL(k_pipe_vblend_mfma<false>, dim3((uint32_t)nb), dim3(256), rows, st, tmp, bg, dst, coefs,
-                           descs, ftyb, max_ov_w);
+                           descs, ftyb, max_ov_w, trim, tstride);
     IPP_CHECK_LAUNCH();
     return IPP_OK;
 }
@@ -1167,11 +1202,23 @@
                                      int32_t max_ov_w, int32_t max_ov_h, int32_t tap_format, void* stream) {
     if (n_images == 0) return IPP_OK;
     if (!bg) return IPP_E_ARG;
-    return vblend_entry(tmp, bg, dst, coefs, descs, n_images, bg_w, bg_h, max_ov_w, max_ov_h, tap_format, stream);
+    return vblend_entry(tmp, bg, dst, coefs, descs, n_images, bg_w, bg_h, max_ov_w, max_ov_h, tap_format, nullptr, 0,
+                        stream);
+}
+
+extern "C" int ipp_pipe_vblend_bands_trim(const uint8_t* tmp, const uint8_t* bg, uint8_t* dst, const int32_t* coefs,
+                                          const ipp_pipe_desc* descs, int32_t n_images, int32_t bg_w, int32_t bg_h,
+                                          int32_t max_ov_w, int32_t max_ov_h, int32_t tap_format,
+                                          const uint16_t* trim, int32_t max_rows, void* stream) {
+    if (n_images == 0) return IPP_OK;
+    if (!bg) return IPP_E_ARG;
+    return vblend_entry(tmp, bg, dst, coefs, descs, n_images, bg_w, bg_h, max_ov_w, max_ov_h, tap_format, trim,
+                        max_rows, stream);
 }
 
 extern "C" int ipp_pipe_vblend_over(const uint8_t* tmp, uint8_t* dst, const int32_t* coefs,
                                     const ipp_pipe_desc* descs, int32_t n_images, int32_t bg_w, int32_t bg_h,
                                     int32_t max_ov_w, int32_t max_ov_h, int32_t tap_format, void* stream) {
-    return vblend_entry(tmp, nullptr, dst, coefs, descs, n_images, bg_w, bg_h, max_ov_w, max_ov_h, tap_format, stream);
-}
+    return vblend_entry(tmp, nullptr, dst, coefs, descs, n_images, bg_w, bg_h, max_ov_w, max_ov_h, tap_format, nullptr,
+                        0, stream);
+}
diff --git a/image_processor_pipeline_amd/csrc/ipp_pipe_layout.h b/image_processor_pipeline_amd/csrc/ipp_pipe_layout.h
--- a/image_processor_pipeline_amd/csrc/ipp_pipe_layout.h
+++ b/image_processor_pipeline_amd/csrc/ipp_pipe_layout.h
@@ -66,6 +66,22 @@
     return (((int64_t)(rows + 15) / 16) * 16 + kKStepCols * nkb_v + 16) / kTGroupRows;
 }
 
+constexpr int kTrimOpen = 255;
+constexpr uint32_t kTrimNone = kTrimOpen << 8;
+constexpr uint32_t kTrimAll = 0;
+IPP_HD constexpr int trim_bands(int max_rows) { return (max_rows + kBandRows - 1) / kBandRows; }
+IPP_HD constexpr uint32_t trim_entry(int lo, int hi) { return (uint32_t)lo | (uint32_t)imin(hi, kTrimOpen) << 8; }
+IPP_HD constexpr bool trim_const(uint32_t e, int ct) {
+    return ct < (int)(e & 255u) || (ct >= (int)(e >> 8 & 255u) && (e >> 8 & 255u) != (uint32_t)kTrimOpen);
+}
+IPP_HD constexpr int trim_v_band(int k0, int ks, int lane) { return (k0 >> 4) + (kKStepCols / kBandRows) * ks + (lane >> 4); }
+static_assert(kKStepCols == 4 * kBandRows && kBandRows == 4 * kTGroupRows,
+              "a V lane's four groups of a K step are one H band, a K step is four");
+static_assert(trim_const(trim_entry(2, 5), 1) && !trim_const(trim_entry(2, 5), 2) && !trim_const(trim_entry(2, 5), 4) &&
+                  trim_const(trim_entry(2, 5), 5) && trim_const(kTrimAll, 0) && !trim_const(kTrimNone, 300) &&
+                  !trim_const(trim_entry(0, 300), 299),
+              "trim_const");
+
 static_assert(tap_block_word(1) == 20 && tap_bias_word(1) == 4, "blocks begin at word 20·T, bias at 4·T (ipp.h)");
 static_assert((1 << kTileOutLog2) == kTileOut && (1 << kTGroupRowsLog2) == kTGroupRows, "the shifts");
 static_assert(kKStepBytes == 3072, "3072 bytes per K step (ipp.h, ipp_plan_mfma_tile)");
diff --git a/image_processor_pipeline_amd/fused.py b/image_processor_pipeline_amd/fused.py
--- a/image_processor_pipeline_amd/fused.py
+++ b/image_processor_pipeline_amd/fused.py
@@ -244,16 +244,22 @@
     return b
 
 
+def trim_bands(plan: PipePlan) -> int:
+    return (plan.max_rows + 15) // 16
+
+
 def _launch_hpass_bgcopy(lib, plan: PipePlan, src: int, tmp: int, coefs: int, descs: int, n: int, bgs: int, out: int,
-                         stream: int) -> None:
-    N.check(lib.ipp_pipe_hpass_bgcopy(src, tmp, coefs, descs, n, plan.max_out_w, plan.max_rows, 3, N.np_ptr(plan.hsv),
-                                      plan.tap_format, bgs, out, stream), "ipp_pipe_hpass_bgcopy")
+                         stream: int, trim: Optional[int] = None) -> None:
+    N.check(lib.ipp_pipe_hpass_bgcopy_trim(src, tmp, coefs, descs, n, plan.max_out_w, plan.max_rows, 3,
+                                           N.np_ptr(plan.hsv), plan.tap_format, bgs, out, trim, stream),
+            "ipp_pipe_hpass_bgcopy_trim")
 
 
 def _launch_vblend_bands(lib, plan: PipePlan, tmp: int, bgs: int, out: int, coefs: int, descs: int, n: int,
-                         stream: int) -> None:
-    N.check(lib.ipp_pipe_vblend_bands(tmp, bgs, out, coefs, descs, n, plan.bg_w, plan.bg_h, plan.max_ov_w,
-                                      plan.max_ov_h, plan.tap_format, stream), "ipp_pipe_vblend_bands")
+                         stream: int, trim: Optional[int] = None) -> None:
+    N.check(lib.ipp_pipe_vblend_bands_trim(tmp, bgs, out, coefs, descs, n, plan.bg_w, plan.bg_h, plan.max_ov_w,
+                                           plan.max_ov_h, plan.tap_format, trim, plan.max_rows, stream),
+            "ipp_pipe_vblend_bands_trim")
 
 
 class _Runner:
@@ -265,11 +271,15 @@
         self.descs = _to_dev(plan.descs, self.device)
         self.coefs, self.host_tiles = plan_taps(pipe, self.device)
         self.tmp = torch.empty(pipe.tmp_bytes, dtype=torch.uint8, device=self.device)
+        self.trim = torch.empty((len(plan.descs), trim_bands(pipe)), dtype=torch.int16, device=self.device)
         self.lib = N.load()
         self._hpass_done = False
 
     def _dptr(self, d0: int) -> int:
         return self.descs.data_ptr() + d0 * self.plan.descs.itemsize
+
+    def _tptr(self, d0: int) -> int:
+        return self.trim.data_ptr() + d0 * self.trim.stride(0) * self.trim.element_size()
 
     def _check_tensors(self, caller: str, src: torch.Tensor, bgs: torch.Tensor, out: torch.Tensor) -> None:
         who = f"{type(self).__name__}.{caller}"
@@ -289,7 +299,8 @@
         p = self.plan
         i0, n = items if items is not None else (0, len(p.descs))
         _launch_hpass_bgcopy(self.lib, p, src.data_ptr(), self.tmp.data_ptr(), self.coefs.data_ptr(),
-                             self._dptr(i0), n, bgs.data_ptr(), out.data_ptr(), _stream(self.device))
+                             self._dptr(i0), n, bgs.data_ptr(), out.data_ptr(), _stream(self.device),
+                             trim=self._tptr(i0))
         self._hpass_done = True
 
     def overlay_bboxes(self, alpha_min: int = 1, items=None) -> np.ndarray:
@@ -305,9 +316,10 @@
             raise N.NativeError("PipeRunner.overlay_bboxes: no H launch (hpass_bgcopy) has run on this runner")
         p = self.plan
         bbox = torch.empty(4 * max(n, 0), dtype=torch.int32, device=self.device)
-        N.check(self.lib.ipp_pipe_overlay_bbox(self.tmp.data_ptr(), self.coefs.data_ptr(), self._dptr(i0), n,
-                                               p.max_ov_w, p.max_ov_h, alpha_min, p.tap_format, bbox.data_ptr(),
-                                               _stream(self.device)), "ipp_pipe_overlay_bbox")
+        N.check(self.lib.ipp_pipe_overlay_bbox_trim(self.tmp.data_ptr(), self.coefs.data_ptr(), self._dptr(i0), n,
+                                                    p.max_ov_w, p.max_ov_h, alpha_min, p.tap_format, bbox.data_ptr(),
+                                                    self._tptr(i0), p.max_rows, _stream(self.device)),
+                "ipp_pipe_overlay_bbox_trim")
         return bbox
 
     def _bboxes_by_item(self, bbox: torch.Tensor, i0: int, n: int) -> np.ndarray:
@@ -321,7 +333,7 @@
         p = self.plan
         i0, n = items if items is not None else (0, len(p.descs))
         _launch_vblend_bands(self.lib, p, self.tmp.data_ptr(), bgs.data_ptr(), out.data_ptr(), self.coefs.data_ptr(),
-                             self._dptr(i0), n, _stream(self.device))
+                             self._dptr(i0), n, _stream(self.device), trim=self._tptr(i0))
 
     def run_overlapped(self, src: torch.Tensor, bgs: torch.Tensor, out: torch.Tensor, parts: int,
                        ratio: float = 1.0) -> None:
@@ -404,6 +416,7 @@
         bufs = {"descs": self._buf(slot, "descs", plan.descs.nbytes),
                 "coefs": self._buf(slot, "coefs", 4 * (plan.coef_words + 4096)),
                 "tmp": self._buf(slot, "tmp", plan.tmp_bytes),
+                "trim": self._buf(slot, "trim", 2 * len(plan.descs) * trim_bands(plan)),
                 "scratch": self._buf(slot, "scratch", self.lib.ipp_pipe_taps_scratch_bytes(len(plan.axes)))}
         stats = np.zeros(2, np.int64)
         side = slot["side"]
@@ -438,9 +451,10 @@
                     ev[0].record(main)
                 _launch_hpass_bgcopy(self.lib, plan, src.data_ptr(), b["tmp"].data_ptr(), b["coefs"].data_ptr(),
                                      b["descs"].data_ptr(), len(plan.descs), bgs.data_ptr(), out.data_ptr(),
-                                     main.cuda_stream)
+                                     main.cuda_stream, trim=b["trim"].data_ptr())
                 _launch_vblend_bands(self.lib, plan, b["tmp"].data_ptr(), bgs.data_ptr(), out.data_ptr(),
-                                     b["coefs"].data_ptr(), b["descs"].data_ptr(), len(plan.descs), main.cuda_stream)
+                                     b["coefs"].data_ptr(), b["descs"].data_ptr(), len(plan.descs), main.cuda_stream,
+                                     trim=b["trim"].data_ptr())
                 if ev:
                     ev[1].record(main)
                     self.events.append(ev)
diff --git a/include/ipp.h b/include/ipp.h
--- a/include/ipp.h
+++ b/include/ipp.h
@@ -144,6 +144,21 @@
 int ipp_pipe_overlay_bbox(const uint8_t* tmp, const int32_t* coefs, const ipp_pipe_desc* descs,
                           int32_t n_images, int32_t max_ov_w, int32_t max_ov_h,
                           int32_t alpha_min, int32_t tap_format, int32_t* bbox, void* stream);
+
+int ipp_pipe_hpass_bgcopy_trim(const uint8_t* src, uint8_t* tmp, const int32_t* coefs,
+                               const ipp_pipe_desc* descs, int32_t n_images,
+                               int32_t max_out_w, int32_t max_rows, int32_t src_cn,
+                               const ipp_hsv_params* hsv, int32_t tap_format,
+                               const uint8_t* bg, uint8_t* dst, uint16_t* trim, void* stream);
+int ipp_pipe_vblend_bands_trim(const uint8_t* tmp, const uint8_t* bg, uint8_t* dst,
+                               const int32_t* coefs, const ipp_pipe_desc* descs, int32_t n_images,
+                               int32_t bg_w, int32_t bg_h, int32_t max_ov_w, int32_t max_ov_h,
+                               int32_t tap_format, const uint16_t* trim, int32_t max_rows,
+                               void* stream);
+int ipp_pipe_overlay_bbox_trim(const uint8_t* tmp, const int32_t* coefs, const ipp_pipe_desc* descs,
+                               int32_t n_images, int32_t max_ov_w, int32_t max_ov_h,
+                               int32_t alpha_min, int32_t tap_format, int32_t* bbox,
+                               const uint16_t* trim, int32_t max_rows, void* stream);
 
 int ipp_pipe_hpass(const uint8_t* src, uint8_t* tmp, const int32_t* coefs,
                    const ipp_pipe_desc* descs, int32_t n_images, int32_t max_out_w,
```

After: 474,200 (median of 6 runs). 3.4% higher.
